# zhenyuw16/Uni3DETR

Measured on AMD Instinct MI355X. Metric: scenes/sec (fwd+bwd) SUN-RGB-D 20k pts, 300 queries, higher is better.
Workload: dtype bf16

## Files before the change

include/u3d_hip.h:

```cpp
#ifndef U3D_HIP_H_
#define U3D_HIP_H_

#include <stddef.h>
#include <stdint.h>

#ifdef __cplusplus
extern "C" {
#endif

typedef struct ihipStream_t* u3d_stream;

enum {
  U3D_OK = 0,
  U3D_ERR_ARG = -1,
  U3D_ERR_UNSUPPORTED = -2,
  U3D_ERR_LAUNCH = -3,
  U3D_ERR_WORKSPACE = -4
};

enum { U3D_F32 = 0, U3D_BF16 = 1 };

int32_t u3d_version(void);
const char* u3d_strerror(int32_t code);

int32_t u3d_event_create(void** event);
int32_t u3d_event_record(void* event, int32_t external, u3d_stream s);
int32_t u3d_event_elapsed_ms(void* start, void* stop, float* ms);
int32_t u3d_event_destroy(void* event);

typedef struct u3d_bitgrid {
  void* words;
  void* prefix;
  int32_t batch, dz, dy, dx;
  int32_t layout;
  int32_t row_capacity;
} u3d_bitgrid;

int64_t u3d_bitgrid_nwords(int32_t batch, int32_t dz, int32_t dy, int32_t dx);
int64_t u3d_bitgrid_nwords_layout(int32_t batch, int32_t dz, int32_t dy, int32_t dx, int32_t layout);

int32_t u3d_bitgrid_mark(const u3d_bitgrid* g, const int32_t* coors, int32_t n, u3d_stream s);

int32_t u3d_bitgrid_mark_strided(const u3d_bitgrid* g, const int32_t* in_coors, const int32_t* n_dev,
                                 int32_t n_cap, const int32_t ksize[3], const int32_t stride[3],
                                 const int32_t pad[3], u3d_stream s);

int64_t u3d_bitgrid_scan_scratch(int64_t nwords);
int32_t u3d_bitgrid_scan(const u3d_bitgrid* g, void* scratch, u3d_stream s);

int32_t u3d_bitgrid_rank(const u3d_bitgrid* g, const int32_t* coors, int32_t n, int32_t* rank, u3d_stream s);

int32_t u3d_bitgrid_coords(const u3d_bitgrid* g, int32_t* coors_out, int32_t cap, u3d_stream s);

int32_t u3d_nbr_table(const u3d_bitgrid* target, const int32_t* q_coors, const int32_t* n_dev, int32_t n_cap,
                      const int32_t ksize[3], const int32_t stride[3], const int32_t pad[3], int32_t mode,
                      int32_t* nbr, int32_t ld, u3d_stream s);

int32_t u3d_dense_nbr_table(int32_t batch, const int32_t q_dims[3], const int32_t t_dims[3], const int32_t ksize[3],
                            const int32_t stride[3], const int32_t pad[3], int32_t mode, int32_t* nbr, int32_t ld,
                            u3d_stream s);

int64_t u3d_voxelize_hard_workspace(int32_t n_total, int32_t batch, int32_t max_pts_per_scene);
int32_t u3d_voxelize_hard(const float* points, const int32_t* scene_off, int32_t batch, int32_t n_total,
                          int32_t max_pts_per_scene, int32_t nfeat, const float voxel_size[3],
                          const float pc_range[6], int32_t max_points, int32_t max_voxels,
                          float* voxels, int32_t* coors, int32_t* num_points, float* mean,
                          int32_t* voxel_off, void* workspace, int64_t workspace_bytes, u3d_stream s);

int32_t u3d_voxelize_dynamic(const float* points, const int32_t* scene_off, int32_t batch, int32_t n_total, int32_t nfeat,
                             const float voxel_size[3], const float pc_range[6], int32_t* coors, u3d_stream s);
int32_t u3d_scatter_mean(const float* points, const int32_t* rank, int32_t n_total, int32_t nfeat, float* sums,
                         int32_t* counts, int32_t n_voxels, u3d_stream s);

int32_t u3d_spconv_fwd(const void* in, const void* w, const int32_t* nbr, int32_t ld, void* out,
                       const int32_t* n_out_dev, int32_t n_out_cap, int32_t cin, int32_t cout, int32_t kvol,
                       int32_t transpose_w, int32_t dtype, u3d_stream s);

int32_t u3d_igemm_fwd_bf16(const void* in, const void* w, const int32_t* nbr, int32_t ld, void* out,
                           const int32_t* n_out_dev, int32_t n_out_cap, int32_t cin, int32_t cout, int32_t kvol,
                           int32_t transpose_w, u3d_stream s);
int32_t u3d_igemm_fwd_add_bf16(const void* in, const void* w, const int32_t* nbr, int32_t ld, const void* addend, void* out,
                               const int32_t* n_out_dev, int32_t n_out_cap, int32_t cin, int32_t cout, int32_t kvol,
                               int32_t transpose_w, u3d_stream s);
int32_t u3d_linear_bf16(const void* x, const void* w, const float* bias, int32_t relu, void* out, const int32_t* m_dev,
                        int32_t m_cap, int32_t k, int32_t n, u3d_stream s);
int64_t u3d_bn_fold_job_bytes(void);
int32_t u3d_bn_fold_job_blocks(int32_t kvol, int32_t cout, int32_t cin);
int32_t u3d_bn_fold_batched(const void* jobs, int32_t njobs, int32_t total_blocks, u3d_stream s);
int32_t u3d_igemm_fwd_affine_bf16(const void* in, const void* w_folded, const int32_t* nbr, int32_t ld, const float* shift, int32_t relu,
                                  void* out, const int32_t* n_out_dev, int32_t n_out_cap, int32_t cin, int32_t cout, int32_t kvol,
                                  u3d_stream s);
int32_t u3d_igemm_fwd_affine_plan(int32_t n_out_cap, int32_t cin, int32_t cout, int32_t kvol, int32_t has_nbr, int32_t* kernel,
                                  int32_t* rows, int32_t* cols);
int32_t u3d_igemm_fwd_split_bf16(const void* in, const void* w, const int32_t* nbr, int32_t ld, float* out, const int32_t* n_out_dev,
                                 int32_t n_out_cap, int32_t cin, int32_t cout, int32_t kvol3, double* stats, const float* addend, u3d_stream s);
int32_t u3d_igemm_direct_split_bf16(const void* in, const void* w3, const int32_t* nbr, int32_t ld, float* out, const int32_t* n_out_dev,
                                    int32_t n_out_cap, int32_t n_in_cap, int32_t cin, int32_t cout, u3d_stream s);
int32_t u3d_igemm_direct_affine_bf16(const void* in, const void* w_folded, const int32_t* nbr, int32_t ld, const float* shift,
                                     int32_t relu, const void* addend, void* out, const int32_t* n_out_dev, int32_t n_out_cap,
                                     int32_t cin, int32_t cout, u3d_stream s);
int32_t u3d_split3_weights(const float* src, int64_t sk, int64_t sa, int64_t sb, int32_t k, int32_t a, int32_t b, void* dst, u3d_stream s);
typedef struct U3dSplitRowsJobs {
  const float* src[32];
  void* dst[32];
  int32_t ld[32], rows[32], cols[32];
  int32_t first_block[33];
  int32_t njobs;
} U3dSplitRowsJobs;
int32_t u3d_split_rows_batch(const U3dSplitRowsJobs* jobs, u3d_stream s);
int32_t u3d_sum3_f32(const float* a, const float* b, const float* c, float* out, int64_t n, u3d_stream s);
int64_t u3d_split3_job_bytes(void);
int32_t u3d_split3_job_blocks(int32_t k, int32_t a, int32_t b);
int32_t u3d_split3_weights_batch(const void* jobs, int32_t njobs, int32_t total_blocks, u3d_stream s);
int32_t u3d_split_rows_f32(const float* x, const int32_t* n_dev, int32_t n_cap, int32_t c, void* dst, u3d_stream s);
int32_t u3d_igemm_fwd_stats_bf16(const void* in, const void* w, const int32_t* nbr, int32_t ld, void* out,
                                 const int32_t* n_out_dev, int32_t n_out_cap, int32_t cin, int32_t cout, int32_t kvol,
                                 double* stats, u3d_stream s);
int32_t u3d_igemm_fwd_stats_layout(int32_t n_out_cap, int32_t cin, int32_t cout, int32_t kvol, int32_t has_nbr, int32_t* partials,
                                   int32_t* rows_per_partial);
typedef struct {
  const void* x;
  const void* y;
  const float* mean;
  const float* invstd;
  const float* gamma;
  const float* beta;
  int32_t relu;
  int32_t reserved;
} u3d_bn_epi;
int32_t u3d_igemm_dgrad_bnstats_bf16(const void* in, const void* w, const int32_t* nbr, int32_t ld, const void* addend, void* out,
                                     const int32_t* n_out_dev, int32_t n_out_cap, int32_t cin, int32_t cout, int32_t kvol,
                                     const u3d_bn_epi* bn, double* stats, u3d_stream s);
int32_t u3d_bn_bwd_finalize_partials(const double* partial, int32_t nblocks, int32_t rows_per_block, const int32_t* n_dev,
                                     int32_t n_cap, int32_t c, double* sums, float* sums_f32, u3d_stream s);
int32_t u3d_subm_halo_sizes(int32_t n_cap, int64_t* tile_rows_elems, int64_t* loc_elems, int32_t* tiles);
int32_t u3d_subm_halo_build(const int32_t* nbr, int32_t ld, const int32_t* n_dev, int32_t n_cap, int32_t* tile_rows,
                            uint16_t* loc, int32_t* tile_cnt, int32_t kvol, u3d_stream s);
int32_t u3d_subm_halo_wpack(const void* w_nmajor, void* w_packed, u3d_stream s);
int32_t u3d_subm_halo_wpack_batched(const void* const* srcs_dev, void* const* dsts_dev, int32_t n, u3d_stream s);
int32_t u3d_subm_halo_conv64_bf16(const void* in, const void* w_packed, const int32_t* tile_rows, const uint16_t* loc,
                                  const int32_t* tile_cnt, const int32_t* n_dev, int32_t n_cap, int32_t krev,
                                  const void* addend, void* out, double* stats, const u3d_bn_epi* bn, int32_t max_slots,
                                  u3d_stream s);
int32_t u3d_subm_halo_wpack128(const void* w_nmajor, void* w_packed, int32_t kvol, u3d_stream s);
int32_t u3d_subm_halo_wpack128_batched(const void* const* srcs_dev, void* const* dsts_dev, int32_t n, int32_t kvol, u3d_stream s);
int32_t u3d_subm_halo_conv128_bf16(const void* in, const void* w_packed, const int32_t* tile_rows, const uint16_t* loc,
                                   const int32_t* tile_cnt, const int32_t* n_dev, int32_t n_cap, int32_t krev,
                                   const void* addend, void* out, double* stats, int32_t max_slots, int32_t kvol, u3d_stream s);
int32_t u3d_subm_halo_conv64_affine_bf16(const void* in, const void* w_packed, const int32_t* tile_rows, const uint16_t* loc,
                                         const int32_t* tile_cnt, const int32_t* n_dev, int32_t n_cap, const void* addend, void* out,
                                         const float* shift, int32_t relu, int32_t max_slots, u3d_stream s);
int32_t u3d_subm_halo_conv128_affine_bf16(const void* in, const void* w_packed, const int32_t* tile_rows, const uint16_t* loc,
                                          const int32_t* tile_cnt, const int32_t* n_dev, int32_t n_cap, const void* addend, void* out,
                                          const float* shift, int32_t relu, int32_t max_slots, int32_t kvol, u3d_stream s);
int64_t u3d_subm_halo_wgrad64_workspace(void);
int32_t u3d_subm_halo_wgrad64_bf16(const void* x, const void* dy, const int32_t* tile_rows, const uint16_t* loc,
                                   const int32_t* tile_cnt, const int32_t* n_dev, int32_t n_cap, float* dw, void* workspace,
                                   int64_t workspace_bytes, int32_t max_slots, u3d_stream s);
int64_t u3d_igemm_wgrad_bf16_workspace(int32_t n_out_cap, int32_t cin, int32_t cout, int32_t kvol);
int32_t u3d_igemm_wgrad_bf16(const void* in, const void* dout, const int32_t* nbr, int32_t ld, float* dw,
                             const int32_t* n_out_dev, int32_t n_out_cap, int32_t cin, int32_t cout, int32_t kvol,
                             int32_t out_layout, void* workspace, int64_t workspace_bytes, u3d_stream s);
int32_t u3d_igemm_wgrad_plan(int32_t n_out_cap, int32_t cin, int32_t cout, int32_t kvol, int32_t has_nbr, int32_t out_layout,
                             int32_t* kernel, int32_t* tile, int32_t* nsplit, int64_t* workspace);

int64_t u3d_spconv_wgrad_workspace(int32_t n_out_cap, int32_t cin, int32_t cout, int32_t kvol);
int32_t u3d_spconv_wgrad(const void* in, const void* dout, const int32_t* nbr, int32_t ld, float* dw,
                         const int32_t* n_out_dev, int32_t n_out_cap, int32_t cin, int32_t cout, int32_t kvol,
                         int32_t dtype, void* workspace, int64_t workspace_bytes, u3d_stream s);

int64_t u3d_colsum_workspace(int32_t n, int32_t c);
int32_t u3d_colsum(const void* x, int32_t n, int32_t c, int32_t dtype, float* out, void* workspace,
                   int64_t workspace_bytes, u3d_stream s);

int64_t u3d_wgrad_batched_workspace(int32_t count, int32_t n_rows, int32_t cin, int32_t cout);
int32_t u3d_wgrad_batched_bf16(const void* const* in, const void* const* dout, float* const* dw, int32_t count,
                               const int32_t* n_dev, int32_t n_rows, int32_t cin, int32_t cout, void* workspace,
                               int64_t workspace_bytes, u3d_stream s);
int64_t u3d_colsum_batched_workspace(int32_t count, int32_t n, int32_t c);
int32_t u3d_colsum_batched(const void* const* x, float* const* out, int32_t count, int32_t n, int32_t c, int32_t dtype,
                           void* workspace, int64_t workspace_bytes, u3d_stream s);

int32_t u3d_skinny_wgrad_chunks(int32_t m);
int32_t u3d_skinny_wgrad_bf16(const void* dy, const void* x, int32_t m, int32_t n, int32_t k, float* partial, u3d_stream s);
int32_t u3d_skinny_wgrad_batched(const void* const* dy, const void* const* x, float* const* partial, const int32_t* n, const int32_t* k,
                                 int32_t count, int32_t m, int32_t dy_skinny, u3d_stream s);

int64_t u3d_bn_stats_workspace(int32_t n_cap, int32_t c);
int32_t u3d_bn_stats(const void* x, const int32_t* n_dev, int32_t n_cap, int32_t c, int32_t dtype,
                     double* sums, void* workspace, int64_t workspace_bytes, u3d_stream s);
int32_t u3d_bn_finalize(const double* sums, const int32_t* n_dev, int32_t n_cap, int32_t c, float eps, float momentum,
                        float* running_mean, float* running_var, int64_t* num_batches, float* mean, float* invstd,
                        u3d_stream s);
int32_t u3d_bn_forward_stats(const void* x, const int32_t* n_dev, int32_t n_cap, int32_t c, int32_t dtype, float eps,
                             float momentum, float* running_mean, float* running_var, int64_t* num_batches, float* mean,
                             float* invstd, void* workspace, int64_t workspace_bytes, u3d_stream s);
int32_t u3d_bn_finalize_partials(const double* partial, int32_t nblocks, int32_t rows_per_block, const int32_t* n_dev,
                                 int32_t n_cap, int32_t c, float eps, float momentum, float* running_mean, float* running_var,
                                 int64_t* num_batches, float* mean, float* invstd, u3d_stream s);
int32_t u3d_bn_apply(const void* x, const float* mean, const float* invstd, const float* gamma,
                     const float* beta, const void* residual, int32_t relu, void* y,
                     const int32_t* n_dev, int32_t n_cap, int32_t c, int32_t dtype, const int32_t* row_map, const void* post_add,
                     u3d_stream s);
int32_t u3d_bn_bwd_stats(const void* dy, const void* y, const void* x, const float* mean, const float* invstd,
                         const float* gamma, const float* beta, int32_t relu, const int32_t* n_dev, int32_t n_cap,
                         int32_t c, int32_t dtype, double* sums, void* workspace, int64_t workspace_bytes,
                         const int32_t* row_map, float* sums_f32, u3d_stream s);
int32_t u3d_bn_bwd_apply(const void* dy, const void* y, const void* x, const float* mean, const float* invstd,
                         const float* gamma, const float* beta, const double* sums, int32_t relu, void* dx, void* dres,
                         const int32_t* n_dev, int32_t n_cap, int32_t c, int32_t dtype, const int32_t* row_map, u3d_stream s);
int32_t u3d_bn_apply_planes(const float* x, const float* mean, const float* invstd, const float* gamma, const float* beta,
                            const float* residual, int32_t relu, float* y, void* planes, const int32_t* n_dev, int32_t n_cap,
                            int32_t c, const int32_t* row_map, const float* post_add, u3d_stream s);
int32_t u3d_bn_bwd_apply_planes(const float* dy, const float* y, const float* x, const float* mean, const float* invstd,
                                const float* gamma, const float* beta, const double* sums, int32_t relu, float* dx, float* dres,
                                void* planes, const int32_t* n_dev, int32_t n_cap, int32_t c, const int32_t* row_map, u3d_stream s);

int32_t u3d_to_dense(const void* feat, const int32_t* coors, const int32_t* n_dev, int32_t n_cap, int32_t c,
                     void* dense, int32_t dz, int32_t dy, int32_t dx, int32_t dtype, u3d_stream s);
int32_t u3d_from_dense(const void* dense, const int32_t* coors, const int32_t* n_dev, int32_t n_cap, int32_t c,
                       void* feat, int32_t dz, int32_t dy, int32_t dx, int32_t dtype, u3d_stream s);

int32_t u3d_gather_rows(const void* in, const int32_t* idx, int32_t n, int32_t row_bytes, void* out, u3d_stream s);
int32_t u3d_scatter_rows(const void* in, const int32_t* idx, int32_t n, int32_t row_bytes, void* out, u3d_stream s);

int32_t u3d_fps(const float* base, const int64_t* set_off, const int32_t* set_n, int32_t nsets, int32_t max_n,
                int32_t m, int32_t* out_idx, float* temp, int64_t temp_stride, int32_t* err, int64_t poll_ticks, int32_t max_wg,
                u3d_stream s);
int32_t u3d_fps2(const float* base, const float* base2, int32_t split, const int64_t* set_off, const int32_t* set_n,
                 int32_t nsets, int32_t max_n, int32_t m, int32_t* out_idx, float* temp, int64_t temp_stride, int32_t* err,
                 int64_t poll_ticks, int32_t max_wg, u3d_stream s);
int32_t u3d_fps_prep(const int32_t* coors, int32_t v_rows, const int32_t* scene_off, const int32_t* voxel_off, int32_t batch,
                     int32_t nfeat, float* vox, int64_t* set_off, int32_t* set_n, u3d_stream s);
int32_t u3d_fps_points(const float* pts, int32_t nfeat, const float* vox, const int32_t* idx, const int32_t* scene_off,
                       const int32_t* voxel_off, int32_t batch, int32_t m, float* out, u3d_stream s);
int32_t u3d_query_embed_fwd(const float* tgt, const float* anchor, const float* fps, const float* rnd, int32_t batch, int32_t nq,
                            int32_t groups, int32_t c, float* query_embeds, float* query, float* ref, float* ref_sig, u3d_stream s);
int32_t u3d_query_embed_bwd(const float* d_query_embeds, const float* d_query, const float* d_ref, const float* d_ref_sig,
                            const float* anchor, int32_t batch, int32_t nq, int32_t groups, int32_t c, float* d_tgt, float* d_anchor,
                            u3d_stream s);

int32_t u3d_match_cost(const float* cls, const float* box, const float* gt, const int32_t* labels,
                       const int32_t* gt_off, int32_t nlayers, int32_t batch, int32_t nq_total, int32_t ncls,
                       int32_t code_size, int32_t gmax, float w_cls, float w_reg, float w_iou, float alpha,
                       float gamma, float* cost, u3d_stream s);
int32_t u3d_lsa(const float* cost, const int32_t* gt_off, int32_t nlayers, int32_t batch, int32_t nq_total,
                int32_t nq, int32_t gmax, int32_t* assigned, u3d_stream s);

int32_t u3d_trilinear_fwd(const void* value, const float* grid, int32_t batch, int32_t nq, int32_t dz, int32_t dy, int32_t dx,
                          int32_t c, void* out, int32_t dtype, u3d_stream s);
int32_t u3d_trilinear_bwd(const void* value, const float* grid, const void* dout, int32_t batch, int32_t nq, int32_t dz,
                          int32_t dy, int32_t dx, int32_t c, float* dvalue, float* dgrid, int32_t dtype, u3d_stream s);

int32_t u3d_iou3d_rotated_aligned(const float* a, const float* b, int32_t n, float* out, u3d_stream s);

int64_t u3d_nms3d_workspace(int32_t n);
int32_t u3d_nms3d(const float* boxes, const int32_t* labels, int32_t n, float thr, uint8_t* keep, void* workspace,
                  int64_t workspace_bytes, u3d_stream s);

#define U3D_DET_TAIL_NONE 0
#define U3D_DET_TAIL_NMS 1
#define U3D_DET_TAIL_DECODE 2
#define U3D_DET_TAIL_MAX_K 8192
#define U3D_DET_TAIL_LDS_CAP 2048
int64_t u3d_det_tail_workspace(int32_t batch, int32_t nq, int32_t num_classes, int32_t max_num, int32_t box_dim);
int32_t u3d_det_tail(const float* prob, const float* fused, const float* boxes, int32_t batch, int32_t nq, int32_t num_classes,
                     int32_t box_dim, int32_t max_num, const float* center_range, float score_threshold, int32_t mode, float nms_thr,
                     const float* score_thr, int32_t num_thr, float* out_boxes, float* out_scores, int32_t* out_labels,
                     int32_t* out_count, int32_t* out_off, void* workspace, int64_t workspace_bytes, u3d_stream s);

#define U3D_DET_TAIL_SOFT_NMS 3
#define U3D_DET_TAIL_MERGE 4
int64_t u3d_det_tail_pp_workspace(int32_t batch, int32_t nq, int32_t num_classes, int32_t max_num, int32_t box_dim, int32_t mode);
int32_t u3d_det_tail_pp(const float* prob, const float* fused, const float* boxes, int32_t batch, int32_t nq, int32_t num_classes,
                        int32_t box_dim, int32_t max_num, const float* center_range, float score_threshold, int32_t mode, float nms_thr,
                        const float* score_thr, int32_t num_thr, float soft_sigma, float soft_prune, float* out_boxes, float* out_scores,
                        int32_t* out_labels, int32_t* out_count, int32_t* out_off, void* workspace, int64_t workspace_bytes, u3d_stream s);

int32_t u3d_tap_gather_sum(const void* p, const int32_t* nbr, int32_t ld, const int32_t* n_dev, int32_t n_cap, int32_t c,
                           int32_t kvol, int32_t dtype, void* out, u3d_stream s);
int32_t u3d_tap_gather_sum_add(const void* p, const int32_t* nbr, int32_t ld, const int32_t* n_dev, int32_t n_cap, int32_t c,
                               int32_t kvol, int32_t dtype, const void* addend, void* out, u3d_stream s);

int32_t u3d_layernorm_blocks(int32_t n);
int32_t u3d_layernorm_fwd(const void* x, int32_t x_dtype, int32_t n, int32_t c, const float* gamma, const float* beta,
                          float eps, int32_t relu, void* y, int32_t y_dtype, float* mean, float* rstd, u3d_stream s);
int32_t u3d_layernorm_bwd(const void* dy, int32_t y_dtype, const void* x, int32_t x_dtype, int32_t n, int32_t c,
// ... 281 lines not shown
```

uni3detr_amd/csrc/geometry.hip:

```cpp
#include "common.h"

extern "C" int64_t u3d_bitgrid_nwords(int32_t batch, int32_t dz, int32_t dy, int32_t dx) {
  return (int64_t)batch * ((dz + 3) / 4) * ((dy + 3) / 4) * ((dx + 3) / 4);
}
extern "C" int64_t u3d_bitgrid_nwords_layout(int32_t batch, int32_t dz, int32_t dy, int32_t dx, int32_t layout) {
  if (layout == 1) return ((int64_t)batch * dz * dy * dx + 63) / 64;
  return u3d_bitgrid_nwords(batch, dz, dy, dx);
}
static inline long long grid_nwords(const u3d_bitgrid* g) { return u3d_bitgrid_nwords_layout(g->batch, g->dz, g->dy, g->dx, g->layout); }

__global__ void k_bitgrid_mark(BitGridDev g, unsigned long long* words, const int4* __restrict__ coors, int n) {
  int i = blockIdx.x * blockDim.x + threadIdx.x;
  if (i >= n) return;
  int4 c = coors[i];
  if (c.x < 0 || c.x >= g.B) return;
  if ((unsigned)c.y >= (unsigned)g.Dz || (unsigned)c.z >= (unsigned)g.Dy || (unsigned)c.w >= (unsigned)g.Dx) return;
  atomicOr(&words[u3d_word_index(g, c.x, c.y, c.z, c.w)], 1ull << u3d_bit_index(g, c.x, c.y, c.z, c.w));
}

extern "C" int32_t u3d_bitgrid_mark(const u3d_bitgrid* g, const int32_t* coors, int32_t n, u3d_stream s) {
  U3D_REQUIRE(g && g->words && coors, U3D_ERR_ARG);
  if (n <= 0) return U3D_OK;
  BitGridDev d = u3d_make_grid(g);
  hipLaunchKernelGGL(k_bitgrid_mark, dim3(u3d_cdiv(n, 256)), dim3(256), 0, s, d, (unsigned long long*)g->words,
// ... 188 lines not shown
  hipLaunchKernelGGL(k_scan_final, dim3(nchunks), dim3(SCAN_TPB), 0, s, (const unsigned long long*)g->words, nwords,
                     (const unsigned*)cs, (unsigned*)g->prefix, nchunks);
  U3D_CHECK_LAUNCH();
  return U3D_OK;
}

__global__ void k_bitgrid_rank(BitGridDev g, const int4* __restrict__ coors, int n, int* __restrict__ rank) {
  int i = blockIdx.x * blockDim.x + threadIdx.x;
  if (i >= n) return;
  int4 c = coors[i];
  rank[i] = (c.x < 0 || c.x >= g.B) ? -1 : u3d_grid_lookup(g, c.x, c.y, c.z, c.w);
}

extern "C" int32_t u3d_bitgrid_rank(const u3d_bitgrid* g, const int32_t* coors, int32_t n, int32_t* rank, u3d_stream s) {
  U3D_REQUIRE(g && g->words && g->prefix && coors && rank, U3D_ERR_ARG);
  if (n <= 0) return U3D_OK;
  hipLaunchKernelGGL(k_bitgrid_rank, dim3(u3d_cdiv(n, 256)), dim3(256), 0, s, u3d_make_grid(g), (const int4*)coors, n, rank);
  U3D_CHECK_LAUNCH();
  return U3D_OK;
}

__global__ void k_bitgrid_coords(BitGridDev g, long long nwords, int4* __restrict__ out, int cap) {
  long long w = (long long)blockIdx.x * blockDim.x + threadIdx.x;
  {
    const int count = g.prefix[nwords];
    for (long long i = w; i < cap; i += (long long)gridDim.x * blockDim.x)
      if (i >= count) out[i] = make_int4(-1, -1, -1, -1);
  }
  if (w >= nwords) return;
  unsigned long long bits = g.words[w];
  if (!bits) return;
  unsigned r = g.prefix[w];
  if (g.linear) {
    while (bits) {
      int bit = __ffsll((long long)bits) - 1;
      bits &= bits - 1;
      long long t = w * 64 + bit;
      int x = (int)(t % g.Dx); t /= g.Dx;
      int y = (int)(t % g.Dy); t /= g.Dy;
      int z = (int)(t % g.Dz); t /= g.Dz;
      if ((int)r < cap) out[r] = make_int4((int)t, z, y, x);
      ++r;
    }
    return;
  }
  long long t = w;
  int bx = (int)(t % g.bx); t /= g.bx;
  int by = (int)(t % g.by); t /= g.by;
  int bz = (int)(t % g.bz); t /= g.bz;
  int b = (int)t;
  while (bits) {
    int bit = __ffsll((long long)bits) - 1;
    bits &= bits - 1;
    if ((int)r < cap) out[r] = make_int4(b, bz * 4 + (bit >> 4), by * 4 + ((bit >> 2) & 3), bx * 4 + (bit & 3));
    ++r;
  }
}

extern "C" int32_t u3d_bitgrid_coords(const u3d_bitgrid* g, int32_t* coors_out, int32_t cap, u3d_stream s) {
  U3D_REQUIRE(g && g->words && g->prefix && coors_out, U3D_ERR_ARG);
  long long nwords = grid_nwords(g);
  hipLaunchKernelGGL(k_bitgrid_coords, dim3(u3d_cdiv(nwords, 256)), dim3(256), 0, s, u3d_make_grid(g), nwords,
                     (int4*)coors_out, cap);
  U3D_CHECK_LAUNCH();
  return U3D_OK;
}

__global__ void k_nbr_table(BitGridDev g, const int4* __restrict__ q, const int* __restrict__ n_dev, int n_cap,
                            Conv3 cv, int mode, int* __restrict__ nbr, int ld) {
  int i = blockIdx.x * blockDim.x + threadIdx.x;
  if (i >= ld) return;
  int n = min(*n_dev, n_cap);
  int kvol = cv.k[0] * cv.k[1] * cv.k[2];
  if (i >= n) {
    for (int k = 0; k < kvol; ++k) nbr[(long long)k * ld + i] = -1;
    return;
  }
  int4 c = q[i];
  int k = 0;
  for (int kz = 0; kz < cv.k[0]; ++kz)
    for (int ky = 0; ky < cv.k[1]; ++ky)
      for (int kx = 0; kx < cv.k[2]; ++kx, ++k) {
        int r = -1;
        if (mode == 0) {
          r = u3d_grid_lookup(g, c.x, c.y * cv.s[0] - cv.p[0] + kz, c.z * cv.s[1] - cv.p[1] + ky, c.w * cv.s[2] - cv.p[2] + kx);
        } else {
          int tz = c.y + cv.p[0] - kz, ty = c.z + cv.p[1] - ky, tx = c.w + cv.p[2] - kx;
          if (tz >= 0 && ty >= 0 && tx >= 0 && tz % cv.s[0] == 0 && ty % cv.s[1] == 0 && tx % cv.s[2] == 0)
            r = u3d_grid_lookup(g, c.x, tz / cv.s[0], ty / cv.s[1], tx / cv.s[2]);
        }
        nbr[(long long)k * ld + i] = r;
      }
}

extern "C" int32_t u3d_nbr_table(const u3d_bitgrid* target, const int32_t* q_coors, const int32_t* n_dev, int32_t n_cap,
                                 const int32_t ksize[3], const int32_t stride[3], const int32_t pad[3], int32_t mode,
                                 int32_t* nbr, int32_t ld, u3d_stream s) {
  U3D_REQUIRE(target && target->words && target->prefix && q_coors && n_dev && nbr, U3D_ERR_ARG);
  U3D_REQUIRE(ld >= n_cap && (mode == 0 || mode == 1), U3D_ERR_ARG);
  if (ld <= 0) return U3D_OK;
  Conv3 cv;
  for (int i = 0; i < 3; ++i) { cv.k[i] = ksize[i]; cv.s[i] = stride[i]; cv.p[i] = pad[i]; U3D_REQUIRE(stride[i] > 0 && ksize[i] > 0, U3D_ERR_ARG); }
  hipLaunchKernelGGL(k_nbr_table, dim3(u3d_cdiv(ld, 256)), dim3(256), 0, s, u3d_make_grid(target), (const int4*)q_coors,
                     n_dev, n_cap, cv, mode, nbr, ld);
  U3D_CHECK_LAUNCH();
  return U3D_OK;
}

__global__ void k_dense_nbr_table(int B, int qz, int qy, int qx, int tz, int ty, int tx, Conv3 cv, int mode,
                                  int* __restrict__ nbr, int ld) {
  int i = blockIdx.x * blockDim.x + threadIdx.x;
  if (i >= ld) return;
  int kvol = cv.k[0] * cv.k[1] * cv.k[2];
  long long nq = (long long)B * qz * qy * qx;
  if (i >= nq) {
    for (int k = 0; k < kvol; ++k) nbr[(long long)k * ld + i] = -1;
    return;
  }
  int x = i % qx; int t = i / qx;
  int y = t % qy; t /= qy;
  int z = t % qz; int b = t / qz;
  int k = 0;
  for (int kz = 0; kz < cv.k[0]; ++kz)
    for (int ky = 0; ky < cv.k[1]; ++ky)
      for (int kx = 0; kx < cv.k[2]; ++kx, ++k) {
        int pz, py, px;
        bool ok = true;
        if (mode == 0) {
          pz = z * cv.s[0] - cv.p[0] + kz; py = y * cv.s[1] - cv.p[1] + ky; px = x * cv.s[2] - cv.p[2] + kx;
        } else {
          int uz = z + cv.p[0] - kz, uy = y + cv.p[1] - ky, ux = x + cv.p[2] - kx;
          ok = uz >= 0 && uy >= 0 && ux >= 0 && uz % cv.s[0] == 0 && uy % cv.s[1] == 0 && ux % cv.s[2] == 0;
          pz = uz / cv.s[0]; py = uy / cv.s[1]; px = ux / cv.s[2];
        }
        ok = ok && (unsigned)pz < (unsigned)tz && (unsigned)py < (unsigned)ty && (unsigned)px < (unsigned)tx;
        nbr[(long long)k * ld + i] = ok ? (int)((((long long)b * tz + pz) * ty + py) * tx + px) : -1;
      }
}

extern "C" int32_t u3d_dense_nbr_table(int32_t batch, const int32_t q_dims[3], const int32_t t_dims[3], const int32_t ksize[3],
                                       const int32_t stride[3], const int32_t pad[3], int32_t mode, int32_t* nbr, int32_t ld,
                                       u3d_stream s) {
  U3D_REQUIRE(nbr && batch > 0 && (mode == 0 || mode == 1), U3D_ERR_ARG);
  long long nq = (long long)batch * q_dims[0] * q_dims[1] * q_dims[2];
  U3D_REQUIRE(ld >= nq && nq < 0x7fffffffll, U3D_ERR_ARG);
  Conv3 cv;
  for (int i = 0; i < 3; ++i) { cv.k[i] = ksize[i]; cv.s[i] = stride[i]; cv.p[i] = pad[i]; U3D_REQUIRE(stride[i] > 0 && ksize[i] > 0, U3D_ERR_ARG); }
  hipLaunchKernelGGL(k_dense_nbr_table, dim3(u3d_cdiv(ld, 256)), dim3(256), 0, s, batch, q_dims[0], q_dims[1], q_dims[2],
                     t_dims[0], t_dims[1], t_dims[2], cv, mode, nbr, ld);
  U3D_CHECK_LAUNCH();
  return U3D_OK;
}

__global__ void k_gather_rows(const uint32_t* __restrict__ in, const int* __restrict__ idx, int n, int row_words,
                              uint32_t* __restrict__ out) {
  long long t = (long long)blockIdx.x * blockDim.x + threadIdx.x;
  long long total = (long long)n * row_words;
  if (t >= total) return;
  int r = (int)(t / row_words), w = (int)(t % row_words);
  int src = idx[r];
  out[t] = src >= 0 ? in[(long long)src * row_words + w] : 0u;
}
__global__ void k_scatter_rows(const uint32_t* __restrict__ in, const int* __restrict__ idx, int n, int row_words,
                               uint32_t* __restrict__ out) {
  long long t = (long long)blockIdx.x * blockDim.x + threadIdx.x;
  long long total = (long long)n * row_words;
  if (t >= total) return;
  int r = (int)(t / row_words), w = (int)(t % row_words);
  int dst = idx[r];
  if (dst >= 0) out[(long long)dst * row_words + w] = in[t];
}

extern "C" int32_t u3d_gather_rows(const void* in, const int32_t* idx, int32_t n, int32_t row_bytes, void* out, u3d_stream s) {
  U3D_REQUIRE(in && idx && out && row_bytes > 0 && (row_bytes & 3) == 0, U3D_ERR_ARG);
  if (n <= 0) return U3D_OK;
  int rw = row_bytes / 4;
  hipLaunchKernelGGL(k_gather_rows, dim3(u3d_cdiv((long long)n * rw, 256)), dim3(256), 0, s, (const uint32_t*)in, idx, n, rw, (uint32_t*)out);
  U3D_CHECK_LAUNCH();
  return U3D_OK;
}
extern "C" int32_t u3d_scatter_rows(const void* in, const int32_t* idx, int32_t n, int32_t row_bytes, void* out, u3d_stream s) {
  U3D_REQUIRE(in && idx && out && row_bytes > 0 && (row_bytes & 3) == 0, U3D_ERR_ARG);
  if (n <= 0) return U3D_OK;
  int rw = row_bytes / 4;
  hipLaunchKernelGGL(k_scatter_rows, dim3(u3d_cdiv((long long)n * rw, 256)), dim3(256), 0, s, (const uint32_t*)in, idx, n, rw, (uint32_t*)out);
  U3D_CHECK_LAUNCH();
  return U3D_OK;
}

struct VoxCfg {
  float vs[3], lo[3];
  int grid[3];
  int nfeat, max_points, max_voxels, hsize;
};

__device__ __forceinline__ unsigned hash_u32(unsigned k) {
  k ^= k >> 16; k *= 0x7feb352dU; k ^= k >> 15; k *= 0x846ca68bU; k ^= k >> 16;
  return k;
}

__global__ void k_vox_insert(const float* __restrict__ pts, const int* __restrict__ scene_off, int B, int n_total, VoxCfg cfg,
                             unsigned* __restrict__ keys, unsigned* __restrict__ first, int* __restrict__ head,
                             int* __restrict__ next, int* __restrict__ slot_of) {
  int i = blockIdx.x * blockDim.x + threadIdx.x;
  if (i >= n_total) return;
  if (i >= scene_off[B]) { slot_of[i] = -1; next[i] = -1; return; }
  int b = 0;
  while (b + 1 < B && i >= scene_off[b + 1]) ++b;
  int il = i - scene_off[b];
  const float* p = pts + (long long)i * cfg.nfeat;
  int c[3];
  bool ok = true;
#pragma unroll
  for (int j = 0; j < 3; ++j) {
    float q = __fdiv_rn(__fsub_rn(p[j], cfg.lo[j]), cfg.vs[j]);
    bool in = (q >= 0.f) && (q < (float)cfg.grid[j]);
    c[j] = in ? (int)floorf(q) : 0;
    ok = ok && in;
  }
  if (!ok) { slot_of[i] = -1; next[i] = -1; return; }
  unsigned key = ((unsigned)c[2] * (unsigned)cfg.grid[1] + (unsigned)c[1]) * (unsigned)cfg.grid[0] + (unsigned)c[0];
  unsigned mask = (unsigned)cfg.hsize - 1u;
  unsigned h = hash_u32(key) & mask;
  long long tb = (long long)b * cfg.hsize;
  while (true) {
    unsigned prev = atomicCAS(&keys[tb + h], 0xFFFFFFFFu, key);
    if (prev == 0xFFFFFFFFu || prev == key) break;
    h = (h + 1) & mask;
  }
  atomicMin(&first[tb + h], (unsigned)il);
  next[i] = atomicExch(&head[tb + h], il);
  slot_of[i] = (int)h;
}

__global__ void k_vox_rank(const int* __restrict__ scene_off, VoxCfg cfg, const unsigned* __restrict__ first,
                           const int* __restrict__ slot_of, int* __restrict__ vid, int* __restrict__ scene_cnt) {
  __shared__ unsigned wsum[16];
  __shared__ unsigned carry_s;
  int b = blockIdx.x;
  int p0 = scene_off[b], n = scene_off[b + 1] - p0;
  long long tb = (long long)b * cfg.hsize;
  if (threadIdx.x == 0) carry_s = 0;
  __syncthreads();
  int lane = threadIdx.x & 63, wid = threadIdx.x >> 6;
  for (int base = 0; base < n; base += 1024) {
    int il = base + threadIdx.x;
    int sl = -1;
    unsigned flag = 0;
    if (il < n) {
      sl = slot_of[p0 + il];
      if (sl >= 0 && first[tb + sl] == (unsigned)il) flag = 1;
    }
    unsigned long long bal = __ballot(flag);
    unsigned in_wave = __popcll(bal & ((1ull << lane) - 1ull));
    if (lane == 0) wsum[wid] = __popcll(bal);
    __syncthreads();
    unsigned woff = 0, tot = 0;
    for (int w = 0; w < 16; ++w) { unsigned v = wsum[w]; if (w < wid) woff += v; tot += v; }
    unsigned carry = carry_s;
    if (flag) {
      unsigned r = carry + woff + in_wave;
      vid[tb + sl] = (r < (unsigned)cfg.max_voxels) ? (int)r : -1;
    }
    __syncthreads();
    if (threadIdx.x == 0) carry_s = carry + tot;
    __syncthreads();
  }
  if (threadIdx.x == 0) scene_cnt[b] = (int)min(carry_s, (unsigned)cfg.max_voxels);
}

__global__ void k_vox_offsets(const int* __restrict__ scene_cnt, int B, int* __restrict__ voxel_off) {
  if (threadIdx.x == 0 && blockIdx.x == 0) {
    int acc = 0;
    for (int b = 0; b < B; ++b) { voxel_off[b] = acc; acc += scene_cnt[b]; }
    voxel_off[B] = acc;
  }
}

__global__ void k_vox_write(const float* __restrict__ pts, const int* __restrict__ scene_off, int B, int n_total, VoxCfg cfg,
                            const unsigned* __restrict__ keys, const unsigned* __restrict__ first, const int* __restrict__ head,
                            const int* __restrict__ next, const int* __restrict__ slot_of, const int* __restrict__ vid,
                            const int* __restrict__ voxel_off, float* __restrict__ voxels, int4* __restrict__ coors,
                            int* __restrict__ num_points, float* __restrict__ mean) {
  int i = blockIdx.x * blockDim.x + threadIdx.x;
  if (i >= n_total || i >= scene_off[B]) return;
  int sl = slot_of[i];
  if (sl < 0) return;
  int b = 0;
  while (b + 1 < B && i >= scene_off[b + 1]) ++b;
  int p0 = scene_off[b];
  int il = i - p0;
  long long tb = (long long)b * cfg.hsize;
  if (first[tb + sl] != (unsigned)il) return;
  int v = vid[tb + sl];
  if (v < 0) return;
  long long row = (long long)voxel_off[b] + v;
  unsigned key = keys[tb + sl];
  int cx = (int)(key % (unsigned)cfg.grid[0]);
  unsigned t = key / (unsigned)cfg.grid[0];
  int cy = (int)(t % (unsigned)cfg.grid[1]);
  int cz = (int)(t / (unsigned)cfg.grid[1]);
  coors[row] = make_int4(b, cz, cy, cx);
  int last = -1, cnt = 0;
  float acc[8];
  const int nf = cfg.nfeat;
  for (int f = 0; f < 8; ++f) acc[f] = 0.f;
// ... 151 lines not shown
```

uni3detr_amd/csrc/igemm_bf16.hip:

```cpp
#include "igemm_common.h"
#include "conv_in.h"
#include "igemm_direct.h"

struct BnEpi {
  const u16* x = nullptr;
  const u16* y = nullptr;
  const float *mean = nullptr, *invstd = nullptr, *gamma = nullptr, *beta = nullptr;
  int relu = 0, pad = 0;
};
template <int BM, int BN, int NT>
__device__ __forceinline__ void bn_bwd_tile_sums(const BnEpi bn, u16* smem, int m0, int col0, int n_out, int cout, int tile,
                                              double* __restrict__ stats, int tid) {
  constexpr int CPR = BN / 8, SWZ = (CPR - 1) & 15, R = NT / CPR, ROWS = BM / R, BATCH = ROWS < 8 ? ROWS : (ROWS % 8 == 0 ? 8 : (ROWS % 6 == 0 ? 6 : 4));
  static_assert(NT % CPR == 0 && BM % R == 0 && ROWS % BATCH == 0, "tile / thread mismatch");
  const int cc = tid % CPR, r0 = tid / CPR;
  const int col = col0 + cc * 8;
  const bool from_y = bn.relu && bn.y, remask = bn.relu && !bn.y;
  float s0[8], s1[8], mu[8], is[8], ga[8], be[8];
#pragma unroll
  for (int e = 0; e < 8; ++e) { s0[e] = 0.f; s1[e] = 0.f; mu[e] = 0.f; is[e] = 0.f; ga[e] = 0.f; be[e] = 0.f; }
  __syncthreads();
  if (col < cout) {
#pragma unroll
    for (int e = 0; e < 8; ++e) { mu[e] = bn.mean[col + e]; is[e] = bn.invstd[col + e]; }
// ... 276 lines not shown
  const int nstage = kvol * kchunks;

  f32x4 acc[WM][WN];
#pragma unroll
  for (int a = 0; a < WM; ++a)
#pragma unroll
    for (int b = 0; b < WN; ++b) acc[a][b] = (f32x4){0.f, 0.f, 0.f, 0.f};

  const __amdgpu_buffer_rsrc_t in_rs = __builtin_amdgcn_make_buffer_rsrc((void*)in, 0, -1, 0x00020000);
  const __amdgpu_buffer_rsrc_t w_rs = __builtin_amdgcn_make_buffer_rsrc((void*)w, 0, -1, 0x00020000);
  const unsigned row_bytes = (unsigned)cin * 2u;
  const int lrow = lane >> 3, lslot = lane & 7;
  unsigned a_part16[SEGS_A], w_voff[SEGS_W];
  int arow[SEGS_A];
#pragma unroll
  for (int u = 0; u < SEGS_A; ++u) {
    const int r = (wv * SEGS_A + u) * 8 + lrow;
    arow[u] = r;
    a_part16[u] = (unsigned)(lslot ^ ((r >> 1) & 7)) * 16u;
  }
#pragma unroll
  for (int u = 0; u < SEGS_W; ++u) {
    const int r = (wv * SEGS_W + u) * 8 + lrow;
    const int part = lslot ^ ((r >> 1) & 7);
    w_voff[u] = (col0 + r < cout) ? (unsigned)((col0 + r) * cin + part * 8) * 2u : 0xFFFFFFFFu;
  }
  int idx_cur[SEGS_A], idx_nxt[SEGS_A];
  auto load_idx_next = [&](int stage) {
    const int kap = stage % kvol;
#pragma unroll
    for (int u = 0; u < SEGS_A; ++u) {
      int m = m0 + arow[u];
      int mc = m < n_out ? m : n_out - 1;
      idx_nxt[u] = nbr ? nbr[(long long)kap * ld + mc] : mc;
    }
  };
  auto advance_idx = [&]() {
#pragma unroll
    for (int u = 0; u < SEGS_A; ++u) idx_cur[u] = (m0 + arow[u] < n_out) ? idx_nxt[u] : -1;
  };
  auto issue = [&](int st, int buf) {
    const int kap = st % kvol, c0 = (st / kvol) * BK;
    u16* Ab = smem + buf * STAGE_ELEMS + wv * (SEGS_A * 512);
    u16* Wb = smem + buf * STAGE_ELEMS + A_ELEMS + wv * (SEGS_W * 512);
    const unsigned a_soff = (unsigned)c0 * 2u;
    const unsigned w_soff = (unsigned)(kap * cin * cout + c0) * 2u;
#pragma unroll
    for (int u = 0; u < SEGS_A; ++u) {
      unsigned voff = idx_cur[u] >= 0 ? (unsigned)idx_cur[u] * row_bytes + a_part16[u] : 0xFFFFFFFFu;
      __builtin_amdgcn_raw_ptr_buffer_load_lds(in_rs, (lds_void_ptr)(Ab + u * 512), 16, voff, a_soff, 0, 0);
    }
#pragma unroll
    for (int u = 0; u < SEGS_W; ++u)
      __builtin_amdgcn_raw_ptr_buffer_load_lds(w_rs, (lds_void_ptr)(Wb + u * 512), 16, w_voff[u], w_soff, 0, 0);
  };
#if GLDS_FRAG_B128
  auto issue_one = [&](int st, int buf, int q) {
    const int kap = st % kvol, c0 = (st / kvol) * BK;
    if (q < SEGS_A) {
      u16* Ab = smem + buf * STAGE_ELEMS + wv * (SEGS_A * 512);
      unsigned voff = idx_cur[q] >= 0 ? (unsigned)idx_cur[q] * row_bytes + a_part16[q] : 0xFFFFFFFFu;
      __builtin_amdgcn_raw_ptr_buffer_load_lds(in_rs, (lds_void_ptr)(Ab + q * 512), 16, voff, (unsigned)c0 * 2u, 0, 0);
    } else {
      const int u = q - SEGS_A;
      u16* Wb = smem + buf * STAGE_ELEMS + A_ELEMS + wv * (SEGS_W * 512);
      __builtin_amdgcn_raw_ptr_buffer_load_lds(w_rs, (lds_void_ptr)(Wb + u * 512), 16, w_voff[u], (unsigned)(kap * cin * cout + c0) * 2u, 0, 0);
    }
  };
  const int g = lane >> 4, li = lane & 15, fsw = (lane >> 1) & 7;
  int foff[2];
#pragma unroll
  for (int ks = 0; ks < 2; ++ks) foff[ks] = ((ks * 4 + g) ^ fsw) << 3;
  typedef const volatile s16x8 __attribute__((address_space(3))) * lds_vptr;
  auto frag = [&](const u16* rowp, int ks) {
    s16x8 v = *(lds_vptr)(rowp + foff[ks]);
    return __builtin_bit_cast(bf16x8, v);
  };
#else
  const int g = lane >> 4, li = lane & 15, fsw = (lane >> 1) & 7;
  int foff[2][2];
#pragma unroll
  for (int ks = 0; ks < 2; ++ks)
#pragma unroll
    for (int j = 0; j < 2; ++j) foff[ks][j] = (((ks * 4 + (g >> 1) + 2 * j) ^ fsw) << 3) + (g & 1) * 4;
  typedef const volatile s16x4 __attribute__((address_space(3))) * lds_vptr;
  auto frag = [&](const u16* rowp, int ks) {
    s16x4 x = *(lds_vptr)(rowp + foff[ks][0]);
    s16x4 y = *(lds_vptr)(rowp + foff[ks][1]);
    s16x8 v = {x[0], x[1], x[2], x[3], y[0], y[1], y[2], y[3]};
    return __builtin_bit_cast(bf16x8, v);
  };

#endif
  load_idx_next(0);
  advance_idx();
  load_idx_next(1 < nstage ? 1 : 0);
  issue(0, 0);
  __syncthreads();
  for (int st = 0; st < nstage; ++st) {
    const int buf = st & 1;
    const int nx = st + 1 < nstage ? st + 1 : st;
    advance_idx();
    load_idx_next(st + 2 < nstage ? st + 2 : nstage - 1);
#if !GLDS_DMA_SPREAD
    issue(nx, buf ^ 1);
#endif
    const u16* A = smem + buf * STAGE_ELEMS + (wm * WM * 16 + li) * BK;
    const u16* W = smem + buf * STAGE_ELEMS + A_ELEMS + (wn * WN * 16 + li) * BK;
#pragma unroll
    for (int ks = 0; ks < 2; ++ks) {
      bf16x8 af[WM];
#pragma unroll
      for (int a = 0; a < WM; ++a) af[a] = frag(A + a * 16 * BK, ks);
#pragma unroll
      for (int b = 0; b < WN; ++b) {
        bf16x8 bfr = frag(W + b * 16 * BK, ks);
#pragma unroll
        for (int a = 0; a < WM; ++a) acc[a][b] = __builtin_amdgcn_mfma_f32_16x16x32_bf16(bfr, af[a], acc[a][b], 0, 0, 0);
#if GLDS_DMA_SPREAD
        {
          constexpr int NQ = SEGS_A + SEGS_W, NG = (GLDS_DMA_SPREAD == 1) ? 2 * WN : (GLDS_DMA_SPREAD == 3 ? (WN > 1 ? WN / 2 : 1) : (GLDS_DMA_SPREAD == 4 ? WN + WN / 2 : WN));
          constexpr int PER = (NQ + NG - 1) / NG;
          const int grp = ks * WN + b;
          if (grp < NG) {
#pragma unroll
            for (int j = 0; j < PER; ++j)
              if (grp * PER + j < NQ) issue_one(nx, buf ^ 1, grp * PER + j);
          }
          __builtin_amdgcn_sched_barrier(0);
        }
#endif
      }
    }
    __syncthreads();
  }
#define GLDS_EPI_ADDEND (BM != 256 || BN != 256)
#include "glds_epilogue.inc"
#undef GLDS_EPI_ADDEND
}

#ifndef GLDS8_PRIO
#define GLDS8_PRIO 1
#endif
#ifndef GLDS8_BALANCE
#define GLDS8_BALANCE 1
#endif
#ifndef GLDS8_STAGGER
#define GLDS8_STAGGER 1
#endif
template <bool F32OUT = false, int RB = 4>
__device__ __forceinline__ void igemm_glds8_body(const u16* __restrict__ in, const u16* __restrict__ w, const int* __restrict__ nbr,
                                                 int ld, u16* __restrict__ out, const int* __restrict__ n_out_dev, int n_out_cap,
                                                 int cin, int cout, int kvol, const float* __restrict__ bias, int relu,
                                                 double* __restrict__ stats, const BnEpi bn) {
  constexpr int WAVES_M = 2, WAVES_N = 4, WM = 2 * RB, WN = 4, NW = 8;
  constexpr int BM = 64 * RB, BN = 256, BK = 64;
  constexpr int PIECE = 128 * BK;
  constexpr int STAGE_ELEMS = 4 * PIECE;
  extern __shared__ __attribute__((aligned(16))) u16 smem[];

  const int n_out = min(*n_out_dev, n_out_cap);
  const int tile = u3d_xcd_tile(blockIdx.x, (n_out + BM - 1) / BM);
  if (tile < 0) return;
  const int m0 = tile * BM;
  const int col0 = blockIdx.y * BN;
  const int tid = threadIdx.x, lane = tid & 63;
  const int wv = __builtin_amdgcn_readfirstlane(tid >> 6);
  const int wm = wv / WAVES_N, wn = wv % WAVES_N;
  const int nstage = kvol * (cin / BK);

  f32x4 acc[WM][WN];
#pragma unroll
  for (int a = 0; a < WM; ++a)
#pragma unroll
    for (int b = 0; b < WN; ++b) acc[a][b] = (f32x4){0.f, 0.f, 0.f, 0.f};

  const __amdgpu_buffer_rsrc_t in_rs = __builtin_amdgcn_make_buffer_rsrc((void*)in, 0, -1, 0x00020000);
  const __amdgpu_buffer_rsrc_t w_rs = __builtin_amdgcn_make_buffer_rsrc((void*)w, 0, -1, 0x00020000);
  const unsigned row_bytes = (unsigned)cin * 2u;
  const int lrow = lane >> 3, lslot = lane & 7;
  unsigned a_part16[2], w_voff[2][2];
  int arow[2][2];
#pragma unroll
  for (int u = 0; u < 2; ++u) {
    const int r = (wv * 2 + u) * 8 + lrow;
    a_part16[u] = (unsigned)(lslot ^ ((r >> 1) & 7)) * 16u;
#pragma unroll
    for (int sp = 0; sp < 2; ++sp) {
      arow[sp][u] = ((r & 63) < 16 * RB) ? (r >> 6) * (32 * RB) + sp * (16 * RB) + (r & 63) : -1;
      const int tc = (r >> 5) * 64 + sp * 32 + (r & 31);
      w_voff[sp][u] = (col0 + tc < cout) ? (unsigned)((col0 + tc) * cin + (lslot ^ ((r >> 1) & 7)) * 8) * 2u : 0xFFFFFFFFu;
    }
  }
  int idx_cur[2][2], idx_nxt[2][2];
  int mcl[2][2];
#pragma unroll
  for (int sp = 0; sp < 2; ++sp)
#pragma unroll
    for (int u = 0; u < 2; ++u) {
      const int m = m0 + (arow[sp][u] < 0 ? 0 : arow[sp][u]);
      mcl[sp][u] = m < n_out ? m : n_out - 1;
      idx_nxt[sp][u] = mcl[sp][u];
    }
  auto load_idx_next = [&](int stage) {
    const int* row = nbr + (long long)(stage % kvol) * ld;
#pragma unroll
    for (int sp = 0; sp < 2; ++sp)
#pragma unroll
      for (int u = 0; u < 2; ++u) idx_nxt[sp][u] = row[mcl[sp][u]];
  };
  auto advance_idx = [&]() {
#pragma unroll
    for (int sp = 0; sp < 2; ++sp)
#pragma unroll
      for (int u = 0; u < 2; ++u) idx_cur[sp][u] = (arow[sp][u] >= 0 && m0 + arow[sp][u] < n_out) ? idx_nxt[sp][u] : -1;
  };
  auto issue_a = [&](int st, int buf, int sp) {
    const unsigned soff = (unsigned)((st / kvol) * BK) * 2u;
    u16* dst = smem + buf * STAGE_ELEMS + sp * PIECE + wv * 1024;
#pragma unroll
    for (int u = 0; u < 2; ++u) {
      const unsigned voff = idx_cur[sp][u] >= 0 ? (unsigned)idx_cur[sp][u] * row_bytes + a_part16[u] : 0xFFFFFFFFu;
      __builtin_amdgcn_raw_ptr_buffer_load_lds(in_rs, (lds_void_ptr)(dst + u * 512), 16, voff, soff, 0, 0);
    }
  };
  auto issue_b = [&](int st, int buf, int sp) {
    const unsigned soff = (unsigned)((st % kvol) * cin * cout + (st / kvol) * BK) * 2u;
    u16* dst = smem + buf * STAGE_ELEMS + (2 + sp) * PIECE + wv * 1024;
#pragma unroll
    for (int u = 0; u < 2; ++u)
      __builtin_amdgcn_raw_ptr_buffer_load_lds(w_rs, (lds_void_ptr)(dst + u * 512), 16, w_voff[sp][u], soff, 0, 0);
  };
  const int g = lane >> 4, li = lane & 15, fsw = (lane >> 1) & 7;
  int foff[2];
#pragma unroll
  for (int ks = 0; ks < 2; ++ks) foff[ks] = ((ks * 4 + g) ^ fsw) << 3;
  typedef const volatile s16x8 __attribute__((address_space(3))) * lds_vptr;
  auto frag = [&](const u16* rowp, int ks) {
    s16x8 v = *(lds_vptr)(rowp + foff[ks]);
    return __builtin_bit_cast(bf16x8, v);
  };
#if GLDS8_BALANCE
  bf16x8 af2[2][RB][2], bf[2][2][2];
#define G8_AF(SP) af2[SP]
#else
  bf16x8 af1[RB][2], bf[2][2][2];
#define G8_AF(SP) af1
#endif
#define G8_READ_A(BUF, SP)                                                                                   \
  {                                                                                                          \
    const u16* A_ = smem + (BUF) * STAGE_ELEMS + (SP) * PIECE + (wm * 64 + li) * BK;                         \
    _Pragma("unroll") for (int a = 0; a < RB; ++a) {                                                         \
      G8_AF(SP)[a][0] = frag(A_ + a * 16 * BK, 0);                                                           \
      G8_AF(SP)[a][1] = frag(A_ + a * 16 * BK, 1);                                                           \
    }                                                                                                        \
  }
#define G8_READ_B(BUF, SP)                                                                                   \
  {                                                                                                          \
    const u16* B_ = smem + (BUF) * STAGE_ELEMS + (2 + (SP)) * PIECE + (wn * 32 + li) * BK;                   \
    _Pragma("unroll") for (int b = 0; b < 2; ++b) {                                                          \
      bf[SP][b][0] = frag(B_ + b * 16 * BK, 0);                                                              \
      bf[SP][b][1] = frag(B_ + b * 16 * BK, 1);                                                              \
    }                                                                                                        \
  }
#define G8_MMA(SA, SB)                                                                                       \
  {                                                                                                          \
    __builtin_amdgcn_s_setprio(GLDS8_PRIO);                                                                  \
    _Pragma("unroll") for (int ks = 0; ks < 2; ++ks)                                                         \
      _Pragma("unroll") for (int b = 0; b < 2; ++b)                                                          \
        _Pragma("unroll") for (int a = 0; a < RB; ++a)                                                       \
          acc[(SA) * RB + a][(SB) * 2 + b] =                                                                 \
              __builtin_amdgcn_mfma_f32_16x16x32_bf16(bf[SB][b][ks], G8_AF(SA)[a][ks], acc[(SA) * RB + a][(SB) * 2 + b], 0, 0, 0); \
    __builtin_amdgcn_s_setprio(0);                                                                           \
  }
#define G8_BAR()                                  \
  {                                               \
    __builtin_amdgcn_sched_barrier(0);            \
    __builtin_amdgcn_s_barrier();                 \
    __builtin_amdgcn_sched_barrier(0);            \
  }
#define G8_VMCNT8() __builtin_amdgcn_s_waitcnt(0x0F78)

  load_idx_next(0);
  advance_idx();
  issue_a(0, 0, 0); issue_b(0, 0, 0); issue_b(0, 0, 1); issue_a(0, 0, 1);
  load_idx_next(1 < nstage ? 1 : 0);
  advance_idx();
  __builtin_amdgcn_s_waitcnt(0x0F70);
  G8_BAR();
#if GLDS8_BALANCE
  G8_READ_A(0, 0)
#endif
  if (GLDS8_STAGGER && wm == 1) G8_BAR();
  for (int st = 0; st < nstage; ++st) {
    const int buf = st & 1;
    const int nx = st + 1 < nstage ? st + 1 : st;
    load_idx_next(st + 2 < nstage ? st + 2 : nstage - 1);
    __builtin_amdgcn_sched_barrier(0);
    G8_READ_B(buf, 0)
#if !GLDS8_BALANCE
    __builtin_amdgcn_sched_barrier(0);
    G8_READ_A(buf, 0)
#endif
    issue_a(nx, buf ^ 1, 0);
    G8_VMCNT8();
    G8_BAR();
    G8_MMA(0, 0)
    G8_BAR();
    G8_READ_B(buf, 1)
    issue_b(nx, buf ^ 1, 0);
    G8_VMCNT8();
    G8_BAR();
    G8_MMA(0, 1)
    G8_BAR();
    G8_READ_A(buf, 1)
    issue_b(nx, buf ^ 1, 1);
#if GLDS8_BALANCE
    __builtin_amdgcn_s_waitcnt(0x0F74);
#endif
    G8_BAR();
    G8_MMA(1, 1)
    G8_BAR();
#if GLDS8_BALANCE
    G8_READ_A(buf ^ 1, 0)
#endif
    issue_a(nx, buf ^ 1, 1);
    __builtin_amdgcn_sched_barrier(0);
    advance_idx();
    __builtin_amdgcn_s_waitcnt(0x0F74);
    G8_BAR();
    G8_MMA(1, 0)
    G8_BAR();
  }
  if (GLDS8_STAGGER && wm == 0) G8_BAR();
  __builtin_amdgcn_s_waitcnt(0x0F70);
  __syncthreads();
#undef G8_AF
#undef G8_READ_A
#undef G8_READ_B
#undef G8_MMA
#undef G8_BAR
#undef G8_VMCNT8
#define GLDS_EPI_ADDEND 1
#include "glds_epilogue.inc"
#undef GLDS_EPI_ADDEND
}
__global__ __launch_bounds__(512) void k_igemm_glds8_256x256(const u16* in, const u16* w, const int* nbr, int ld, u16* out,
                                                             const int* n_out_dev, int n_out_cap, int cin, int cout, int kvol,
                                                             const float* bias, int relu, double* stats, BnEpi bn) {
  igemm_glds8_body(in, w, nbr, ld, out, n_out_dev, n_out_cap, cin, cout, kvol, bias, relu, stats, bn);
}
__global__ __launch_bounds__(512) void k_igemm_glds8_256x256_f32o(const u16* in, const u16* w, const int* nbr, int ld, u16* out,
                                                                  const int* n_out_dev, int n_out_cap, int cin, int cout, int kvol,
                                                                  const float* bias, int relu, double* stats, BnEpi bn) {
  igemm_glds8_body<true>(in, w, nbr, ld, out, n_out_dev, n_out_cap, cin, cout, kvol, bias, relu, stats, bn);
}
__global__ __launch_bounds__(512) void k_igemm_glds8_192x256(const u16* in, const u16* w, const int* nbr, int ld, u16* out,
                                                             const int* n_out_dev, int n_out_cap, int cin, int cout, int kvol,
                                                             const float* bias, int relu, double* stats, BnEpi bn) {
  igemm_glds8_body<false, 3>(in, w, nbr, ld, out, n_out_dev, n_out_cap, cin, cout, kvol, bias, relu, stats, bn);
}
__global__ __launch_bounds__(512) void k_igemm_glds8_192x256_f32o(const u16* in, const u16* w, const int* nbr, int ld, u16* out,
                                                                  const int* n_out_dev, int n_out_cap, int cin, int cout, int kvol,
                                                                  const float* bias, int relu, double* stats, BnEpi bn) {
  igemm_glds8_body<true, 3>(in, w, nbr, ld, out, n_out_dev, n_out_cap, cin, cout, kvol, bias, relu, stats, bn);
}
static inline bool igemm_rows192(int n_out_cap, int col_blocks) {
  const long long w256 = (long long)u3d_cdiv(n_out_cap, 256) * col_blocks, w192 = (long long)u3d_cdiv(n_out_cap, 192) * col_blocks;
  return (double)u3d_cdiv(w192, 256) * 192.0 * 1.05 < (double)u3d_cdiv(w256, 256) * 256.0;
}

template <bool F32OUT = false, int RB = 4>
__device__ __forceinline__ void igemm_glds8n_body(const u16* __restrict__ in, const u16* __restrict__ w, const int* __restrict__ nbr,
                                                  int ld, u16* __restrict__ out, const int* __restrict__ n_out_dev, int n_out_cap,
                                                  int cin, int cout, int kvol, const float* __restrict__ bias, int relu,
                                                  double* __restrict__ stats, const BnEpi bn) {
  constexpr int WAVES_M = 4, WAVES_N = 2, WM = RB, WN = 4, NW = 8;
  constexpr int BM = 64 * RB, BN = 128, BK = 64;
  constexpr int APIECE = 128 * BK, BPIECE = 64 * BK;
  constexpr int STAGE_ELEMS = 2 * APIECE + 2 * BPIECE;
  extern __shared__ __attribute__((aligned(16))) u16 smem[];

  const int n_out = min(*n_out_dev, n_out_cap);
  const int tile = u3d_xcd_tile(blockIdx.x, (n_out + BM - 1) / BM);
  if (tile < 0) return;
  const int m0 = tile * BM;
  const int col0 = blockIdx.y * BN;
  const int tid = threadIdx.x, lane = tid & 63;
  const int wv = __builtin_amdgcn_readfirstlane(tid >> 6);
  const int grp = wv >> 2, wm = wv >> 1, wn = wv & 1;
  const int nstage = kvol * (cin / BK);

  f32x4 acc[WM][WN];
#pragma unroll
  for (int a = 0; a < WM; ++a)
#pragma unroll
    for (int b = 0; b < WN; ++b) acc[a][b] = (f32x4){0.f, 0.f, 0.f, 0.f};

  const __amdgpu_buffer_rsrc_t in_rs = __builtin_amdgcn_make_buffer_rsrc((void*)in, 0, -1, 0x00020000);
  const __amdgpu_buffer_rsrc_t w_rs = __builtin_amdgcn_make_buffer_rsrc((void*)w, 0, -1, 0x00020000);
  const unsigned row_bytes = (unsigned)cin * 2u;
  const int lrow = lane >> 3, lslot = lane & 7;
  unsigned a_part16[2], w_voff[2];
  int arow[2][2];
#pragma unroll
  for (int u = 0; u < 2; ++u) {
    const int r = (wv * 2 + u) * 8 + lrow;
    a_part16[u] = (unsigned)(lslot ^ ((r >> 1) & 7)) * 16u;
#pragma unroll
    for (int gp = 0; gp < 2; ++gp) arow[gp][u] = ((r & 63) < 16 * RB) ? gp * (32 * RB) + (r >> 6) * (16 * RB) + (r & 63) : -1;
  }
  {
    const int r = wv * 8 + lrow;
#pragma unroll
    for (int t = 0; t < 2; ++t) {
      const int tc = (r >> 5) * 64 + t * 32 + (r & 31);
      w_voff[t] = (col0 + tc < cout) ? (unsigned)((col0 + tc) * cin + (lslot ^ ((r >> 1) & 7)) * 8) * 2u : 0xFFFFFFFFu;
    }
  }
  int idx_cur[2][2], idx_nxt[2][2], mcl[2][2];
#pragma unroll
  for (int gp = 0; gp < 2; ++gp)
#pragma unroll
    for (int u = 0; u < 2; ++u) {
      const int m = m0 + (arow[gp][u] < 0 ? 0 : arow[gp][u]);
      mcl[gp][u] = m < n_out ? m : n_out - 1;
      idx_nxt[gp][u] = mcl[gp][u];
    }
  auto load_idx_next = [&](int stage) {
    const int* row = nbr + (long long)(stage % kvol) * ld;
#pragma unroll
    for (int gp = 0; gp < 2; ++gp)
#pragma unroll
      for (int u = 0; u < 2; ++u) idx_nxt[gp][u] = row[mcl[gp][u]];
  };
  auto advance_idx = [&]() {
#pragma unroll
    for (int gp = 0; gp < 2; ++gp)
#pragma unroll
      for (int u = 0; u < 2; ++u) idx_cur[gp][u] = (arow[gp][u] >= 0 && m0 + arow[gp][u] < n_out) ? idx_nxt[gp][u] : -1;
  };
  auto issue_a = [&](int st, int sl) {
    const unsigned soff = (unsigned)((st / kvol) * BK) * 2u;
#pragma unroll
    for (int gp = 0; gp < 2; ++gp) {
      u16* dst = smem + sl * STAGE_ELEMS + gp * APIECE + wv * 1024;
#pragma unroll
      for (int u = 0; u < 2; ++u) {
        const unsigned voff = idx_cur[gp][u] >= 0 ? (unsigned)idx_cur[gp][u] * row_bytes + a_part16[u] : 0xFFFFFFFFu;
        __builtin_amdgcn_raw_ptr_buffer_load_lds(in_rs, (lds_void_ptr)(dst + u * 512), 16, voff, soff, 0, 0);
      }
    }
  };
  auto issue_b = [&](int st, int sl) {
    const unsigned soff = (unsigned)((st % kvol) * cin * cout + (st / kvol) * BK) * 2u;
#pragma unroll
    for (int t = 0; t < 2; ++t) {
      u16* dst = smem + sl * STAGE_ELEMS + 2 * APIECE + t * BPIECE + wv * 512;
      __builtin_amdgcn_raw_ptr_buffer_load_lds(w_rs, (lds_void_ptr)dst, 16, w_voff[t], soff, 0, 0);
    }
  };
  const int g = lane >> 4, li = lane & 15, fsw = (lane >> 1) & 7;
  int foff[2];
#pragma unroll
  for (int ks = 0; ks < 2; ++ks) foff[ks] = ((ks * 4 + g) ^ fsw) << 3;
  typedef const volatile s16x8 __attribute__((address_space(3))) * lds_vptr;
  auto frag = [&](const u16* rowp, int ks) {
    s16x8 v = *(lds_vptr)(rowp + foff[ks]);
    return __builtin_bit_cast(bf16x8, v);
  };
  bf16x8 af[2][RB][2], bf[2][2][2];
#define N8_READ_A(SL, SET)                                                                                   \
  {                                                                                                          \
    const u16* A_ = smem + (SL) * STAGE_ELEMS + grp * APIECE + (((wv >> 1) & 1) * 64 + li) * BK;             \
    _Pragma("unroll") for (int a = 0; a < RB; ++a) {                                                         \
      af[SET][a][0] = frag(A_ + a * 16 * BK, 0);                                                             \
      af[SET][a][1] = frag(A_ + a * 16 * BK, 1);                                                             \
    }                                                                                                        \
  }
#define N8_READ_B(SL)                                                                                        \
  {                                                                                                          \
    _Pragma("unroll") for (int t = 0; t < 2; ++t) {                                                          \
      const u16* B_ = smem + (SL) * STAGE_ELEMS + 2 * APIECE + t * BPIECE + (wn * 32 + li) * BK;             \
      _Pragma("unroll") for (int b = 0; b < 2; ++b) {                                                        \
        bf[t][b][0] = frag(B_ + b * 16 * BK, 0);                                                             \
        bf[t][b][1] = frag(B_ + b * 16 * BK, 1);                                                             \
      }                                                                                                      \
    }                                                                                                        \
  }
#define N8_MMA(SET, T)                                                                                       \
  {                                                                                                          \
    __builtin_amdgcn_s_setprio(1);                                                                           \
    _Pragma("unroll") for (int ks = 0; ks < 2; ++ks)                                                         \
      _Pragma("unroll") for (int b = 0; b < 2; ++b)                                                          \
        _Pragma("unroll") for (int a = 0; a < RB; ++a)                                                       \
          acc[a][(T) * 2 + b] =                                                                              \
              __builtin_amdgcn_mfma_f32_16x16x32_bf16(bf[T][b][ks], af[SET][a][ks], acc[a][(T) * 2 + b], 0, 0, 0); \
    __builtin_amdgcn_s_setprio(0);                                                                           \
  }
#define N8_BAR()                                  \
  {                                               \
    __builtin_amdgcn_sched_barrier(0);            \
    __builtin_amdgcn_s_barrier();                 \
    __builtin_amdgcn_sched_barrier(0);            \
  }
#define N8_TRIP(SET)                                                                                         \
  {                                                                                                          \
    const int s2 = st + 2 < nstage ? st + 2 : nstage - 1;                                                    \
    load_idx_next(st + 3 < nstage ? st + 3 : nstage - 1);                                                    \
    __builtin_amdgcn_sched_barrier(0);                                                                       \
    N8_READ_B(sl0)                                                                                           \
    issue_a(s2, sl2);                                                                                        \
    __builtin_amdgcn_s_waitcnt(0x0F7A);                                   \
    N8_BAR();                                                                                                \
    N8_MMA(SET, 0)                                                                                           \
    N8_BAR();                                                                                                \
    N8_READ_A(sl1, (SET) ^ 1)                                                                                \
    issue_b(s2, sl2);                                                                                        \
    __builtin_amdgcn_sched_barrier(0);                                                                       \
    advance_idx();                                                                                           \
    __builtin_amdgcn_s_waitcnt(0x0F7A);                                   \
    N8_BAR();                                                                                                \
    N8_MMA(SET, 1)                                                                                           \
    N8_BAR();                                                                                                \
    { const int t_ = sl0; sl0 = sl1; sl1 = sl2; sl2 = t_; }                                                  \
    ++st;                                                                                                    \
  }
  load_idx_next(0);
  advance_idx();
  issue_a(0, 0); issue_b(0, 0);
  load_idx_next(1 < nstage ? 1 : 0);
  advance_idx();
  issue_a(1 < nstage ? 1 : 0, 1); issue_b(1 < nstage ? 1 : 0, 1);
  load_idx_next(2 < nstage ? 2 : nstage - 1);
  advance_idx();
  __builtin_amdgcn_s_waitcnt(0x0F70);
  N8_BAR();
  N8_READ_A(0, 0)
  if (grp == 1) N8_BAR();
  int st = 0, sl0 = 0, sl1 = 1, sl2 = 2;
  while (st + 1 < nstage) {
    N8_TRIP(0)
    N8_TRIP(1)
  }
  if (st < nstage) N8_TRIP(0)
  if (grp == 0) N8_BAR();
  __builtin_amdgcn_s_waitcnt(0x0F70);
  __syncthreads();
#undef N8_READ_A
#undef N8_READ_B
#undef N8_MMA
#undef N8_BAR
#undef N8_TRIP
#define GLDS_EPI_ADDEND 1
#include "glds_epilogue.inc"
#undef GLDS_EPI_ADDEND
}
__global__ __launch_bounds__(512) void k_igemm_glds8_256x128(const u16* in, const u16* w, const int* nbr, int ld, u16* out,
                                                             const int* n_out_dev, int n_out_cap, int cin, int cout, int kvol,
                                                             const float* bias, int relu, double* stats, BnEpi bn) {
  igemm_glds8n_body(in, w, nbr, ld, out, n_out_dev, n_out_cap, cin, cout, kvol, bias, relu, stats, bn);
}
__global__ __launch_bounds__(512) void k_igemm_glds8_256x128_f32o(const u16* in, const u16* w, const int* nbr, int ld, u16* out,
                                                                  const int* n_out_dev, int n_out_cap, int cin, int cout, int kvol,
                                                                  const float* bias, int relu, double* stats, BnEpi bn) {
  igemm_glds8n_body<true>(in, w, nbr, ld, out, n_out_dev, n_out_cap, cin, cout, kvol, bias, relu, stats, bn);
}
__global__ __launch_bounds__(512) void k_igemm_glds8_192x128(const u16* in, const u16* w, const int* nbr, int ld, u16* out,
                                                             const int* n_out_dev, int n_out_cap, int cin, int cout, int kvol,
                                                             const float* bias, int relu, double* stats, BnEpi bn) {
  igemm_glds8n_body<false, 3>(in, w, nbr, ld, out, n_out_dev, n_out_cap, cin, cout, kvol, bias, relu, stats, bn);
}
__global__ __launch_bounds__(512) void k_igemm_glds8_192x128_f32o(const u16* in, const u16* w, const int* nbr, int ld, u16* out,
                                                                  const int* n_out_dev, int n_out_cap, int cin, int cout, int kvol,
                                                                  const float* bias, int relu, double* stats, BnEpi bn) {
  igemm_glds8n_body<true, 3>(in, w, nbr, ld, out, n_out_dev, n_out_cap, cin, cout, kvol, bias, relu, stats, bn);
}
#define U3D_GLDS_KERNEL(NAME, A, B, C, D)                                                                                        \
  __global__ __launch_bounds__(A* B * 64) void NAME(const u16* in, const u16* w, const int* nbr, int ld, u16* out,               \
                                                    const int* n_out_dev, int n_out_cap, int cin, int cout, int kvol,            \
                                                    const float* bias, int relu, double* stats, BnEpi bn) {                      \
    igemm_glds_body<A, B, C, D>(in, w, nbr, ld, out, n_out_dev, n_out_cap, cin, cout, kvol, bias, relu, stats, bn);               \
  }
#define U3D_GLDS_KERNEL_X(NAME, ...) U3D_GLDS_KERNEL(NAME, __VA_ARGS__)
U3D_GLDS_KERNEL_X(k_igemm_glds_256x256, GLDS256_CFG)
U3D_GLDS_KERNEL(k_igemm_glds_256x128, 4, 2, 4, 4)
U3D_GLDS_KERNEL(k_igemm_glds_128x64, 4, 1, 2, 4)
U3D_GLDS_KERNEL(k_igemm_glds_128x128, 2, 2, 4, 4)
#undef U3D_GLDS_KERNEL
#define U3D_GLDS_KERNEL_F32O(NAME, A, B, C, D)                                                                                   \
  __global__ __launch_bounds__(A* B * 64) void NAME(const u16* in, const u16* w, const int* nbr, int ld, u16* out,               \
                                                    const int* n_out_dev, int n_out_cap, int cin, int cout, int kvol,            \
                                                    const float* bias, int relu, double* stats, BnEpi bn) {                      \
    igemm_glds_body<A, B, C, D, true>(in, w, nbr, ld, out, n_out_dev, n_out_cap, cin, cout, kvol, bias, relu, stats, bn);         \
  }
U3D_GLDS_KERNEL_F32O(k_igemm_glds_128x64_f32o, 4, 1, 2, 4)
U3D_GLDS_KERNEL_F32O(k_igemm_glds_128x128_f32o, 2, 2, 4, 4)
#undef U3D_GLDS_KERNEL_F32O
typedef void (*glds_kernel_t)(const u16*, const u16*, const int*, int, u16*, const int*, int, int, int, int, const float*, int, double*, BnEpi);


struct GldsKernel {
  glds_kernel_t bf16, f32;
  int rows, cols, threads;
  size_t lds;
  bool addend;
};
#define GLDS_GEOM(A, B, C, D) A * C * 16, B * D * 16, A * B * 64, (size_t)2 * (A * C * 16 + B * D * 16) * 64 * 2
#define GLDS_GEOM_X(...) GLDS_GEOM(__VA_ARGS__)
enum { G_256x256, G8_256x256, G8_192x256, G8_256x128, G8_192x128, G_256x128, G_128x128, G_128x64, G_COUNT };
static const GldsKernel GLDS_KERNELS[G_COUNT] = {
    {k_igemm_glds_256x256, nullptr, GLDS_GEOM_X(GLDS256_CFG), false},
    {k_igemm_glds8_256x256, k_igemm_glds8_256x256_f32o, 256, 256, 512, 2 * (256 + 256) * 64 * 2, true},
    {k_igemm_glds8_192x256, k_igemm_glds8_192x256_f32o, 192, 256, 512, 2 * (256 + 256) * 64 * 2, true},
    {k_igemm_glds8_256x128, k_igemm_glds8_256x128_f32o, 256, 128, 512, 3 * (256 + 128) * 64 * 2, true},
    {k_igemm_glds8_192x128, k_igemm_glds8_192x128_f32o, 192, 128, 512, 3 * (256 + 128) * 64 * 2, true},
    {k_igemm_glds_256x128, nullptr, GLDS_GEOM(4, 2, 4, 4), true},
    {k_igemm_glds_128x128, k_igemm_glds_128x128_f32o, GLDS_GEOM(2, 2, 4, 4), true},
    {k_igemm_glds_128x64, k_igemm_glds_128x64_f32o, GLDS_GEOM(4, 1, 2, 4), true},
};
#undef GLDS_GEOM_X
#undef GLDS_GEOM

enum FwdEpi { EPI_PLAIN, EPI_BIAS_RELU, EPI_ADD, EPI_F32, EPI_F32_ADD, EPI_STATS, EPI_BN_BWD, EPI_AFFINE };

struct FwdPlan {
  DirectPlan direct;
  glds_kernel_t fn = nullptr;
  int glds = -1, rows = 0;
  dim3 grid;
  int threads = 0;
  size_t lds = 0;
  int partials = 0;
  bool served() const { return fn || direct.slot >= 0; }
};

constexpr int GLDS8N_MIN_KTILES = 48;
constexpr int GLDS8N_MIN_WGS = 160;

static FwdPlan fwd_plan(int n_out_cap, int cin, int cout, int kvol, bool has_nbr, bool nmajor, FwdEpi epi) {
  FwdPlan p;
  if (epi == EPI_PLAIN || epi == EPI_ADD || epi == EPI_STATS) {
    p.direct = u3d_plan_igemm_direct(n_out_cap, cin, cout, kvol, has_nbr, nmajor, epi == EPI_STATS ? DIR_STATS : DIR_BF16);
    if (p.direct.slot >= 0) {
      p.partials = p.direct.partials;
      return p;
    }
  }
  if (!nmajor || cin <= 0 || cout <= 0 || cin % 64 != 0 || cout % 64 != 0 || n_out_cap <= 0) return p;
  const long long tiles256 = u3d_cdiv(n_out_cap, 256);
  const bool r192 = has_nbr && kvol > 1;
  int g;
  if (epi == EPI_BIAS_RELU)
    g = (cout % 256 == 0 && tiles256 * (cout / 256) >= 128) ? G_256x256
        : (cout % 128 == 0 && tiles256 * (cout / 128) >= 128) ? G_256x128 : G_128x64;
  else if (cout % 256 == 0 && tiles256 * (cout / 256) >= 128)
    g = !has_nbr ? G_256x256 : (r192 && igemm_rows192(n_out_cap, cout / 256)) ? G8_192x256 : G8_256x256;
  else if (has_nbr && cout % 128 == 0 && kvol * (cin / 64) >= GLDS8N_MIN_KTILES && tiles256 * (cout / 128) >= GLDS8N_MIN_WGS)
    g = (r192 && igemm_rows192(n_out_cap, cout / 128)) ? G8_192x128 : G8_256x128;
  else
    g = cout % 128 == 0 ? G_128x128 : G_128x64;
  const GldsKernel& k = GLDS_KERNELS[g];
  const bool f32 = epi == EPI_F32 || epi == EPI_F32_ADD;
  if (!k.addend && (epi == EPI_ADD || epi == EPI_F32_ADD || epi == EPI_BN_BWD)) return p;
  p.fn = f32 ? k.f32 : k.bf16;
  if (!p.fn) return p;
  p.glds = g;
  p.rows = k.rows;
  p.grid = dim3(u3d_cdiv(n_out_cap, k.rows), u3d_cdiv(cout, k.cols));
  p.threads = k.threads;
  p.lds = k.lds;
  p.partials = (int)p.grid.x;
  return p;
}

static int fwd_launch(const FwdPlan& p, const void* in, const void* w, const int32_t* nbr, int ld, void* out, const int32_t* n_out_dev,
                      int n_out_cap, int cin, int cout, int kvol, hipStream_t s, const void* bias = nullptr, int relu = 0,
                      double* stats = nullptr, const BnEpi bn = BnEpi{}) {
  if (p.direct.slot >= 0) return u3d_launch_igemm_direct(p.direct, in, w, nbr, ld, out, n_out_dev, n_out_cap, cin, cout, s, bias, stats);
  static unsigned long long lds_mask[G_COUNT][2] = {};
  if (p.lds > 64 * 1024) u3d_allow_lds_impl((const void*)p.fn, (int)p.lds, &lds_mask[p.glds][p.fn == GLDS_KERNELS[p.glds].f32]);
  hipLaunchKernelGGL(p.fn, p.grid, dim3(p.threads), p.lds, s, (const u16*)in, (const u16*)w, nbr, ld, (u16*)out, n_out_dev, n_out_cap, cin,
                     cout, kvol, (const float*)bias, relu, stats, bn);
  return hipGetLastError() == hipSuccess ? U3D_OK : U3D_ERR_LAUNCH;
}

extern "C" int32_t u3d_linear_bf16(const void* x, const void* w, const float* bias, int32_t relu, void* out,
                                   const int32_t* m_dev, int32_t m_cap, int32_t k, int32_t n, u3d_stream s) {
  U3D_REQUIRE(x && w && out && m_dev, U3D_ERR_ARG);
  if (k % 64 != 0 || n % 64 != 0) return U3D_ERR_UNSUPPORTED;
  if (m_cap <= 0) return U3D_OK;
  const FwdPlan p = fwd_plan(m_cap, k, n, 1, false, true, EPI_BIAS_RELU);
  if (!p.served()) return U3D_ERR_UNSUPPORTED;
  return fwd_launch(p, x, w, nullptr, 0, out, m_dev, m_cap, k, n, 1, s, bias, relu ? 1 : 0);
}

extern "C" int32_t u3d_igemm_fwd_affine_bf16(const void* in, const void* w_folded, const int32_t* nbr, int32_t ld, const float* shift,
                                             int32_t relu, void* out, const int32_t* n_out_dev, int32_t n_out_cap, int32_t cin,
                                             int32_t cout, int32_t kvol, u3d_stream s) {
  U3D_REQUIRE(in && w_folded && out && n_out_dev && shift && kvol > 0 && (nbr || kvol == 1), U3D_ERR_ARG);
  if (cin <= 0 || cout <= 0 || cin % 64 != 0 || cout % 64 != 0) return U3D_ERR_UNSUPPORTED;
  if (n_out_cap <= 0) return U3D_OK;
  const FwdPlan p = fwd_plan(n_out_cap, cin, cout, kvol, nbr != nullptr, true, EPI_AFFINE);
  if (!p.served()) return U3D_ERR_UNSUPPORTED;
  return fwd_launch(p, in, w_folded, nbr, ld, out, n_out_dev, n_out_cap, cin, cout, kvol, s, shift, relu ? 1 : 0);
}
extern "C" int32_t u3d_igemm_fwd_affine_plan(int32_t n_out_cap, int32_t cin, int32_t cout, int32_t kvol, int32_t has_nbr, int32_t* kernel,
                                             int32_t* rows, int32_t* cols) {
  U3D_REQUIRE(kernel && rows && cols, U3D_ERR_ARG);
  const FwdPlan p = fwd_plan(n_out_cap, cin, cout, kvol, has_nbr != 0, true, EPI_AFFINE);
  if (!p.served()) return U3D_ERR_UNSUPPORTED;
  *kernel = p.glds;
  *rows = p.rows;
  *cols = GLDS_KERNELS[p.glds].cols;
  return U3D_OK;
}

extern "C" int32_t u3d_igemm_fwd_stats_layout(int32_t n_out_cap, int32_t cin, int32_t cout, int32_t kvol, int32_t has_nbr, int32_t* partials,
                                              int32_t* rows_per_partial) {
  U3D_REQUIRE(partials && rows_per_partial, U3D_ERR_ARG);
  const FwdPlan p = fwd_plan(n_out_cap, cin, cout, kvol, has_nbr != 0, true, EPI_STATS);
  if (!p.served()) return U3D_ERR_UNSUPPORTED;
  *partials = p.partials;
  *rows_per_partial = p.rows;
  return U3D_OK;
}
extern "C" int32_t u3d_igemm_fwd_stats_bf16(const void* in, const void* w, const int32_t* nbr, int32_t ld, void* out,
                                            const int32_t* n_out_dev, int32_t n_out_cap, int32_t cin, int32_t cout, int32_t kvol,
                                            double* stats, u3d_stream s) {
  U3D_REQUIRE(in && w && out && n_out_dev && stats && (nbr || kvol == 1), U3D_ERR_ARG);
  const FwdPlan p = fwd_plan(n_out_cap, cin, cout, kvol, nbr != nullptr, true, EPI_STATS);
  if (!p.served()) return U3D_ERR_UNSUPPORTED;
  return fwd_launch(p, in, w, nbr, ld, out, n_out_dev, n_out_cap, cin, cout, kvol, s, nullptr, 0, stats);
}

extern "C" int32_t u3d_igemm_fwd_split_bf16(const void* in, const void* w, const int32_t* nbr, int32_t ld, float* out,
                                            const int32_t* n_out_dev, int32_t n_out_cap, int32_t cin, int32_t cout, int32_t kvol3,
                                            double* stats, const float* addend, u3d_stream s) {
  U3D_REQUIRE(in && w && out && n_out_dev && nbr && kvol3 > 0, U3D_ERR_ARG);
  if (cin % 64 != 0 || cout % 64 != 0) return U3D_ERR_UNSUPPORTED;
  if (n_out_cap <= 0) return U3D_OK;
  const FwdPlan p = fwd_plan(n_out_cap, cin, cout, kvol3, true, true, addend ? EPI_F32_ADD : EPI_F32);
  if (!p.served()) return U3D_ERR_UNSUPPORTED;
  return fwd_launch(p, in, w, nbr, ld, out, n_out_dev, n_out_cap, cin, cout, kvol3, s, addend, addend ? 2 : 0, stats);
}


extern "C" int32_t u3d_igemm_fwd_add_bf16(const void* in, const void* w, const int32_t* nbr, int32_t ld, const void* addend, void* out,
                                          const int32_t* n_out_dev, int32_t n_out_cap, int32_t cin, int32_t cout, int32_t kvol,
                                          int32_t transpose_w, u3d_stream s) {
  U3D_REQUIRE(in && w && out && addend && n_out_dev && nbr, U3D_ERR_ARG);
  if (n_out_cap <= 0) return U3D_OK;
  const FwdPlan p = fwd_plan(n_out_cap, cin, cout, kvol, true, transpose_w != 0, EPI_ADD);
  if (!p.served()) return U3D_ERR_UNSUPPORTED;
  return fwd_launch(p, in, w, nbr, ld, out, n_out_dev, n_out_cap, cin, cout, kvol, s, addend, 2);
}

extern "C" int32_t u3d_igemm_dgrad_bnstats_bf16(const void* in, const void* w, const int32_t* nbr, int32_t ld, const void* addend, void* out,
                                                const int32_t* n_out_dev, int32_t n_out_cap, int32_t cin, int32_t cout, int32_t kvol,
                                                const u3d_bn_epi* bn, double* stats, u3d_stream s) {
  U3D_REQUIRE(in && w && out && n_out_dev && nbr && bn && bn->x && bn->mean && bn->invstd && stats, U3D_ERR_ARG);
  U3D_REQUIRE(!bn->relu || bn->y || (bn->gamma && bn->beta), U3D_ERR_ARG);
  const FwdPlan p = fwd_plan(n_out_cap, cin, cout, kvol, true, true, EPI_BN_BWD);
  if (!p.served()) return U3D_ERR_UNSUPPORTED;
  BnEpi e;
  e.x = (const u16*)bn->x; e.y = (const u16*)bn->y; e.mean = bn->mean; e.invstd = bn->invstd; e.gamma = bn->gamma; e.beta = bn->beta;
  e.relu = bn->relu;
  return fwd_launch(p, in, w, nbr, ld, out, n_out_dev, n_out_cap, cin, cout, kvol, s, addend, addend ? 2 : 0, stats, e);
}

extern "C" int32_t u3d_igemm_fwd_bf16(const void* in, const void* w, const int32_t* nbr, int32_t ld, void* out,
                                      const int32_t* n_out_dev, int32_t n_out_cap, int32_t cin, int32_t cout, int32_t kvol,
                                      int32_t transpose_w, u3d_stream s) {
  U3D_REQUIRE(in && w && out && n_out_dev && (nbr || kvol == 1), U3D_ERR_ARG);
  if (!transpose_w && convin_shape(cin, cout, kvol))
    return u3d_launch_conv_in_fwd(in, w, nbr, ld, out, n_out_dev, n_out_cap, kvol, s);
  const FwdPlan p = fwd_plan(n_out_cap, cin, cout, kvol, nbr != nullptr, transpose_w != 0, EPI_PLAIN);
  if (p.served()) return fwd_launch(p, in, w, nbr, ld, out, n_out_dev, n_out_cap, cin, cout, kvol, s);
  if (n_out_cap > 0 && cin % 16 == 0 && cout % 16 == 0 && cin <= 64 && cout <= 64 && (cin < 64 || cout < 64)) {
#define IG_SMALL(WNV, BKV)                                                                                                                          \
    return transpose_w ? launch_igemm_fwd<4, 1, IGEMM_SMALL_WM, WNV, false, BKV>(in, w, nbr, ld, out, n_out_dev, n_out_cap, cin, cout, kvol, s)   \
                       : launch_igemm_fwd<4, 1, IGEMM_SMALL_WM, WNV, true, BKV>(in, w, nbr, ld, out, n_out_dev, n_out_cap, cin, cout, kvol, s);
    if (cin == 16 || cin == 32) {
      if (cout == 16) { IG_SMALL(1, 32) }
      if (cout == 32) { IG_SMALL(2, 32) }
      if (cout == 64) { IG_SMALL(4, 32) }
    }
#undef IG_SMALL
  }
  if (cin % 64 != 0 || cout % 64 != 0 || cout < 64) return U3D_ERR_UNSUPPORTED;
  if (n_out_cap <= 0) return U3D_OK;
  if (transpose_w) return U3D_ERR_UNSUPPORTED;
#define IG_CASE(A, B, C, D) return launch_igemm_fwd<A, B, C, D, true>(in, w, nbr, ld, out, n_out_dev, n_out_cap, cin, cout, kvol, s);
  const long long wg256 = (long long)u3d_cdiv(n_out_cap, 256) * (cout / 256 > 0 ? cout / 256 : 1);
  if (cout % 256 == 0 && wg256 < 128) { IG_CASE(4, 2, 4, 4) }
  if (cout >= 256 && cout % 256 == 0) { IG_CASE(2, 4, 8, 4) }
  if (cout >= 128 && cout % 128 == 0) { IG_CASE(4, 2, 4, 4) }
  if (cout % 64 == 0) { IG_CASE(4, 1, 2, 4) }
#undef IG_CASE
  return U3D_ERR_UNSUPPORTED;
}
```

uni3detr_amd/native.py:

```python
import ctypes as C
import os

import numpy as np
import torch

from . import abi

_HERE = os.path.dirname(os.path.abspath(__file__))
LIB_PATH = os.environ.get("U3D_LIB_PATH") or os.path.join(_HERE, "libu3d_hip.so")

_ABI = abi.load()
_K = _ABI.constants


def _struct(c_name, py_name):
    return abi.structure(_ABI.structs[c_name], py_name)


def _slot_names(prefix):
    names = sorted((v, n[len(prefix):]) for n, v in _K.items() if n.startswith(prefix))
    assert [v for v, _ in names] == list(range(len(names))) and names[-1][1] == "COUNT" and _K[prefix + "COUNT"] == len(names) - 1
    return [n for _, n in names[:-1]]


U3D_ERR_UNSUPPORTED = _K["U3D_ERR_UNSUPPORTED"]
F32, BF16 = _K["U3D_F32"], _K["U3D_BF16"]


class U3DError(RuntimeError):
    pass


BitGridStruct = _struct("u3d_bitgrid", "BitGridStruct")

for _n, _v in _K.items():
    if _n.startswith(("U3D_DL_", "U3D_DLN_")):
        globals()[_n[4:]] = _v
DS_NAMES = _slot_names("U3D_DS_")
DG_NAMES = _slot_names("U3D_DG_")
DecLayerParams = _struct("u3d_declayer_params", "DecLayerParams")
DecLayerDims = _struct("u3d_declayer_dims", "DecLayerDims")
WPackDesc = _struct("u3d_wpack_desc", "WPackDesc")

_lib = None
_I3 = C.c_int32 * 3
_F3 = C.c_float * 3
_F6 = C.c_float * 6


def exported_symbols():
    return sorted(_ABI.prototypes)


def lib():
    global _lib
    if _lib is None:
        if not os.path.exists(LIB_PATH):
            raise U3DError(f"{LIB_PATH} is missing: run `python -m uni3detr_amd.build` (hipcc, gfx950). "
                           "There is no CPU/PyTorch fallback for the HIP hot path.")
        l = C.CDLL(LIB_PATH)
        for name, (res, args) in _ABI.prototypes.items():
            fn = getattr(l, name)
            fn.restype = res
            fn.argtypes = args
        _lib = l
    return _lib


def _check(rc, what):
    if rc != 0:
        raise U3DError(f"{what} failed: {lib().u3d_strerror(rc).decode()} ({rc})")


def _stream():
    return C.c_void_p(torch.cuda.current_stream().cuda_stream)


def _ptr(t):
    if t is None:
        return None
    assert t.is_cuda and t.is_contiguous(), "device-contiguous tensor required"
    return C.c_void_p(t.data_ptr())


def dtype_code(t):
    if t.dtype == torch.float32:
        return F32
    if t.dtype == torch.bfloat16:
        return BF16
    raise U3DError(f"unsupported dtype {t.dtype}")


class BitGrid:

    def __init__(self, batch, dims, device, linear=False):
        self.batch, self.dims = int(batch), tuple(int(d) for d in dims)
        self.linear = bool(linear)
        self.nwords = int(lib().u3d_bitgrid_nwords_layout(self.batch, *self.dims, 1 if linear else 0))
        self.words = torch.zeros(self.nwords, dtype=torch.int64, device=device)
        self.prefix = torch.empty(self.nwords + 1, dtype=torch.int32, device=device)
        self._scratch = torch.empty(int(lib().u3d_bitgrid_scan_scratch(self.nwords)), dtype=torch.int32, device=device)
        self.c = BitGridStruct(self.words.data_ptr(), self.prefix.data_ptr(), self.batch, *self.dims, 1 if linear else 0, 0)

    def set_row_capacity(self, cap):
        self.c.row_capacity = int(cap)

    def mark(self, coors):
        _check(lib().u3d_bitgrid_mark(C.byref(self.c), _ptr(coors), coors.shape[0], _stream()), "bitgrid_mark")

    def mark_strided(self, in_coors, n_dev, ksize, stride, pad):
        _check(lib().u3d_bitgrid_mark_strided(C.byref(self.c), _ptr(in_coors), _ptr(n_dev), in_coors.shape[0],
                                              _I3(*ksize), _I3(*stride), _I3(*pad), _stream()), "bitgrid_mark_strided")

    def scan(self):
        _check(lib().u3d_bitgrid_scan(C.byref(self.c), _ptr(self._scratch), _stream()), "bitgrid_scan")

    @property
    def count_dev(self):
        return self.prefix[self.nwords:]

    def rank(self, coors):
        out = torch.empty(coors.shape[0], dtype=torch.int32, device=coors.device)
        _check(lib().u3d_bitgrid_rank(C.byref(self.c), _ptr(coors), coors.shape[0], _ptr(out), _stream()), "bitgrid_rank")
        return out

    def coords(self, n):
        out = torch.empty((n, 4), dtype=torch.int32, device=self.words.device)
        _check(lib().u3d_bitgrid_coords(C.byref(self.c), _ptr(out), n, _stream()), "bitgrid_coords")
        return out

    def nbr_table(self, q_coors, n_dev, ksize, stride, pad, mode):
        n = q_coors.shape[0]
        ld = (n + 127) // 128 * 128
        kvol = ksize[0] * ksize[1] * ksize[2]
        nbr = torch.empty((kvol, ld), dtype=torch.int32, device=q_coors.device)
        _check(lib().u3d_nbr_table(C.byref(self.c), _ptr(q_coors), _ptr(n_dev), n, _I3(*ksize), _I3(*stride), _I3(*pad),
                                   mode, _ptr(nbr), ld, _stream()), "nbr_table")
        return nbr


def dense_nbr_table(batch, q_dims, t_dims, ksize, stride, pad, mode, device):
    n = batch * q_dims[0] * q_dims[1] * q_dims[2]
    ld = (n + 127) // 128 * 128
    kvol = ksize[0] * ksize[1] * ksize[2]
    nbr = torch.empty((kvol, ld), dtype=torch.int32, device=device)
    with torch.cuda.device(device):
        _check(lib().u3d_dense_nbr_table(batch, _I3(*q_dims), _I3(*t_dims), _I3(*ksize), _I3(*stride), _I3(*pad), mode, _ptr(nbr), ld,
                                         _stream()), "dense_nbr_table")
    return nbr


def voxelize_hard(points, scene_off, batch, max_pts_per_scene, voxel_size, pc_range, max_points, max_voxels,
                  want_voxels=True, want_mean=True):
    n_total, nfeat = points.shape
    cap = batch * max_voxels
    dev = points.device
    voxels = torch.empty((cap, max_points, nfeat), dtype=torch.float32, device=dev) if want_voxels else None
    coors = torch.full((cap, 4), -1, dtype=torch.int32, device=dev)
    num = torch.zeros((cap,), dtype=torch.int32, device=dev)
    mean = torch.zeros((cap, nfeat), dtype=torch.float32, device=dev) if want_mean else None
    voxel_off = torch.empty((batch + 1,), dtype=torch.int32, device=dev)
    wsb = int(lib().u3d_voxelize_hard_workspace(n_total, batch, max_pts_per_scene))
    ws = torch.empty(wsb, dtype=torch.uint8, device=dev)
    _check(lib().u3d_voxelize_hard(_ptr(points), _ptr(scene_off), batch, n_total, max_pts_per_scene, nfeat,
                                   _F3(*voxel_size), _F6(*pc_range), max_points, max_voxels, _ptr(voxels), _ptr(coors),
                                   _ptr(num), _ptr(mean), _ptr(voxel_off), _ptr(ws), wsb, _stream()), "voxelize_hard")
    return voxels, coors, num, mean, voxel_off


def voxelize_dynamic(points, scene_off, batch, voxel_size, pc_range):
    n_total, nfeat = points.shape
    coors = torch.empty((n_total, 4), dtype=torch.int32, device=points.device)
    _check(lib().u3d_voxelize_dynamic(_ptr(points), _ptr(scene_off), batch, n_total, nfeat, _F3(*voxel_size), _F6(*pc_range),
                                      _ptr(coors), _stream()), "voxelize_dynamic")
    return coors


def scatter_mean(points, rank, n_voxels):
    n_total, nfeat = points.shape
    sums = torch.zeros((n_voxels, nfeat), dtype=torch.float32, device=points.device)
    counts = torch.zeros((n_voxels,), dtype=torch.int32, device=points.device)
    _check(lib().u3d_scatter_mean(_ptr(points), _ptr(rank), n_total, nfeat, _ptr(sums), _ptr(counts), n_voxels, _stream()), "scatter_mean")
    return sums, counts


class ExternalEvent:

    def __init__(self):
        h = C.c_void_p()
        _check(lib().u3d_event_create(C.byref(h)), "event_create")
        self.h = h

    def record(self):
        _check(lib().u3d_event_record(self.h, 1, _stream()), "event_record")

    def elapsed_time(self, other):
        ms = C.c_float()
        _check(lib().u3d_event_elapsed_ms(self.h, other.h, C.byref(ms)), "event_elapsed_ms")
        return float(ms.value)

    def __del__(self):
        try:
            lib().u3d_event_destroy(self.h)
        except Exception:
            pass


class KernelTimer:

    def __init__(self, mode="time", targets=(), per_step=0):
        self.mode, self.calls, self.census = mode, [], []
        self.targets, self.per_step, self.counter, self.marks = set(targets), per_step, 0, {}

    def begin(self):
        if self.mode == "off":
            return None
        if self.mode == "mark":
            i = self.counter % self.per_step if self.per_step else self.counter
            self.counter += 1
            if i not in self.targets:
                return None
            try:
                e = ExternalEvent()
                e.record()
            except U3DError:
                self.mode, self.marks = "off", {}
                return None
            return (i, e)
        e = torch.cuda.Event(enable_timing=True)
        e.record()
        return e

    def end(self, tag, e0, meta=None):
        if self.mode == "off":
            return
        if self.mode == "mark":
            if e0 is not None:
                try:
                    e1 = ExternalEvent()
                    e1.record()
                    self.marks[e0[0]] = (tag, e0[1], e1)
                except U3DError:
                    self.mode, self.marks = "off", {}
            return
        e1 = torch.cuda.Event(enable_timing=True)
        e1.record()
        self.calls.append((tag, e0, e1))
        if self.mode == "census":
            self.census.append((tag, meta))

    def mark_durations_ms(self):
        torch.cuda.synchronize()
        return {i: a.elapsed_time(b) for i, (t, a, b) in self.marks.items()}

    def durations_ms(self):
        torch.cuda.synchronize()
        return [(t, a.elapsed_time(b)) for t, a, b in self.calls]


TIMER = None
CALL_KIND = "sparse"
USE_IGEMM_V2 = True


def census_meta(n_in, n_out, cin, cout, kvol, nbr, act_bytes=2, w_bytes=None, v2=True, split=False):
    if split:
        act_bytes = w_bytes = 4
    elif w_bytes is None:
        w_bytes = act_bytes
    tab = nbr.t if isinstance(nbr, RevNbr) else nbr
    pairs = n_out if tab is None else int((tab[:kvol, :n_out] >= 0).sum().item())
    meta = dict(kind=CALL_KIND, v2=v2, split=True) if split else dict(kind=CALL_KIND, v2=v2)
    meta.update(n_in=n_in, n_out=n_out, cin=cin, cout=cout, kvol=kvol, pairs=pairs,
                bytes=n_in * cin * act_bytes + n_out * cout * act_bytes + 8 * pairs + kvol * cin * cout * w_bytes, flops=2 * pairs * cin * cout)
    return meta


def timed_begin():
    t = TIMER
    return None if t is None else (t, t.begin())


def timed_end(region, tag, *shape, **price):
    if region is not None:
        t, e0 = region
        t.end(tag, e0, census_meta(*shape, **price) if (shape and t.mode == "census") else None)


def fwd_stats_layout(n_out, cin, cout, kvol, has_nbr):
    p, r = C.c_int32(0), C.c_int32(0)
    if lib().u3d_igemm_fwd_stats_layout(n_out, cin, cout, kvol, int(has_nbr), C.byref(p), C.byref(r)) != 0:
        return None
    return p.value, r.value


def spconv_fwd_stats(inp, w_nmajor, nbr, n_out_dev, n_out, cout):
    cin, kvol = inp.shape[1], w_nmajor.shape[0]
    if inp.dtype != torch.bfloat16 or not USE_IGEMM_V2 or (nbr is None and kvol != 1):
        return None
    layout = fwd_stats_layout(n_out, cin, cout, kvol, nbr is not None)
    if layout is None or layout[0] == 0:
        return None
    nblocks, tr = layout
    out = torch.empty((n_out, cout), dtype=inp.dtype, device=inp.device)
    stats = torch.empty((nblocks, 2, cout), dtype=torch.float64, device=inp.device)
    ld = nbr.shape[1] if nbr is not None else 0
    region = timed_begin()
    _check(lib().u3d_igemm_fwd_stats_bf16(_ptr(inp), _ptr(w_nmajor), _ptr(nbr), ld, _ptr(out), _ptr(n_out_dev), n_out, cin, cout, kvol,
                                          _ptr(stats), _stream()), "igemm_fwd_stats_bf16")
    if region is not None:
        timed_end(region, "spconv_fwd", inp.shape[0], n_out, cin, cout, kvol, nbr)
    return out, stats, tr


class BnEpi(_struct("u3d_bn_epi", "_BnEpi")):

    @staticmethod
    def of(x, y, mean, invstd, gamma, beta, relu):
        p = lambda t: None if t is None else t.data_ptr()
        return BnEpi(p(x), p(y), p(mean), p(invstd), p(gamma), p(beta), int(relu), 0)


def spconv_dgrad_bnstats(dout, w_nmajor, nbr, n_dev, n, cout, addend, epi):
    kvol, cin = w_nmajor.shape[0], dout.shape[1]
    if dout.dtype != torch.bfloat16 or not USE_IGEMM_V2 or nbr is None:
        return None
    layout = fwd_stats_layout(n, cin, cout, kvol, True)
    if layout is None or layout[1] == 0:
        return None
    nblocks, tr = layout
    out = torch.empty((n, cout), dtype=dout.dtype, device=dout.device)
    stats = torch.empty((nblocks, 2, cout), dtype=torch.float64, device=dout.device)
    nbr_p, ld = _nbr_ptr_ld(nbr)
    region = timed_begin()
    rc = lib().u3d_igemm_dgrad_bnstats_bf16(_ptr(dout), _ptr(w_nmajor), nbr_p, ld, _ptr(addend), _ptr(out), _ptr(n_dev), n, cin, cout, kvol,
                                            C.byref(epi), _ptr(stats), _stream())
    if rc == U3D_ERR_UNSUPPORTED:
        return None
    _check(rc, "igemm_dgrad_bnstats_bf16")
    if region is not None:
        timed_end(region, "spconv_dgrad", dout.shape[0], n, cin, cout, kvol, nbr)
    return out, stats, tr


def bn_bwd_finalize_partials(partial, tile_rows, n_dev, n_cap):
    nb, _, c = partial.shape
    sums = torch.empty((2, c), dtype=torch.float64, device=partial.device)
    s32 = torch.empty((2, c), dtype=torch.float32, device=partial.device)
    _check(lib().u3d_bn_bwd_finalize_partials(_ptr(partial), nb, tile_rows, _ptr(n_dev), n_cap, c, _ptr(sums), _ptr(s32), _stream()),
           "bn_bwd_finalize_partials")
    return sums, s32


class SubmHalo:
    TILE = 128

    MAX_ROWS = 140 * 256 * 32

    def __init__(self, nbr_fwd, n_dev, n_cap):
        dev = nbr_fwd.device
        a, b, t = C.c_int64(0), C.c_int64(0), C.c_int32(0)
        _check(lib().u3d_subm_halo_sizes(n_cap, C.byref(a), C.byref(b), C.byref(t)), "subm_halo_sizes")
        self.tiles, self.n_dev, self.n_cap, self.nbr = t.value, n_dev, n_cap, nbr_fwd
        self.kvol = nbr_fwd.shape[0]
        self.tile_rows = torch.empty((a.value,), dtype=torch.int32, device=dev)
        self.loc = torch.empty((b.value,), dtype=torch.int16, device=dev)
        self.tile_cnt = torch.empty((t.value,), dtype=torch.int32, device=dev)
        rc = lib().u3d_subm_halo_build(_ptr(nbr_fwd), nbr_fwd.shape[1], _ptr(n_dev), n_cap, _ptr(self.tile_rows), _ptr(self.loc),
                                       _ptr(self.tile_cnt), self.kvol, _stream())
        self.ok = rc != U3D_ERR_UNSUPPORTED
        if self.ok:
            _check(rc, "subm_halo_build")


def subm_halo_wgrad(x, dy, halo, out=None, max_slots=0):
    assert x.dtype == torch.bfloat16 and dy.dtype == torch.bfloat16 and x.shape == dy.shape == (halo.n_cap, 64)
    dw = out.view(27, 64, 64) if (out is not None and out.is_contiguous() and out.dtype == torch.float32 and out.numel() == 27 * 4096) \
        else torch.empty((27, 64, 64), dtype=torch.float32, device=x.device)
    wsb = int(lib().u3d_subm_halo_wgrad64_workspace())
    ws = torch.empty(wsb, dtype=torch.uint8, device=x.device)
    region = timed_begin()
    _check(lib().u3d_subm_halo_wgrad64_bf16(_ptr(x), _ptr(dy), _ptr(halo.tile_rows), _ptr(halo.loc), _ptr(halo.tile_cnt), _ptr(halo.n_dev),
                                            halo.n_cap, _ptr(dw), _ptr(ws), wsb, int(max_slots), _stream()), "subm_halo_wgrad64_bf16")
    if region is not None:
        timed_end(region, "spconv_wgrad", halo.n_cap, halo.n_cap, 64, 64, 27, halo.nbr, w_bytes=4)
    return dw


def subm_halo_wpack(w_nmajor, out=None):
    k, c = w_nmajor.shape[0], w_nmajor.shape[1]
    assert w_nmajor.dtype == torch.bfloat16 and w_nmajor.is_contiguous() and w_nmajor.shape[2] == c
    assert (k == 27 and c == 64) or (1 <= k <= 27 and c == 128)
    out = torch.empty_like(w_nmajor) if out is None else out
    if c == 64:
        _check(lib().u3d_subm_halo_wpack(_ptr(w_nmajor), _ptr(out), _stream()), "subm_halo_wpack")
    else:
        _check(lib().u3d_subm_halo_wpack128(_ptr(w_nmajor), _ptr(out), k, _stream()), "subm_halo_wpack128")
    return out


def subm_halo_wpack_plan(pairs, device):
    k, c = pairs[0][0].shape[0], pairs[0][0].shape[1]
    assert all(tuple(a.shape) == (k, c, c) for a, _ in pairs) and ((k == 27 and c == 64) or c == 128)
    src = torch.tensor([a.data_ptr() for a, _ in pairs], dtype=torch.int64, device=device)
    dst = torch.tensor([b.data_ptr() for _, b in pairs], dtype=torch.int64, device=device)
    return src, dst, len(pairs), pairs, c, k


def subm_halo_wpack_batched(plan):
    if plan[4] == 64:
        _check(lib().u3d_subm_halo_wpack_batched(_ptr(plan[0]), _ptr(plan[1]), plan[2], _stream()), "subm_halo_wpack_batched")
    else:
        _check(lib().u3d_subm_halo_wpack128_batched(_ptr(plan[0]), _ptr(plan[1]), plan[2], plan[5], _stream()), "subm_halo_wpack128_batched")


def subm_halo_conv(inp, w_packed, halo, krev=False, addend=None, want_stats=False, tag="spconv_fwd", bn_epi=None, max_slots=0):
    c = inp.shape[1]
    assert inp.dtype == torch.bfloat16 and c in (64, 128) and tuple(w_packed.shape) == (halo.kvol, c, c) and inp.shape[0] == halo.n_cap
    assert c == 128 or halo.kvol == 27
    assert c == 64 or bn_epi is None, "the BatchNorm-backward epilogue exists on the 64-channel kernel only"
    out = torch.empty_like(inp)
    stats = torch.empty((halo.tiles, 2, c), dtype=torch.float64, device=inp.device) if want_stats else None
    region = timed_begin()
    if c == 64:
        _check(lib().u3d_subm_halo_conv64_bf16(_ptr(inp), _ptr(w_packed), _ptr(halo.tile_rows), _ptr(halo.loc), _ptr(halo.tile_cnt),
                                               _ptr(halo.n_dev), halo.n_cap, int(krev), _ptr(addend), _ptr(out), _ptr(stats),
                                               None if bn_epi is None else C.byref(bn_epi), int(max_slots), _stream()),
               "subm_halo_conv64_bf16")
    else:
        _check(lib().u3d_subm_halo_conv128_bf16(_ptr(inp), _ptr(w_packed), _ptr(halo.tile_rows), _ptr(halo.loc), _ptr(halo.tile_cnt),
                                                _ptr(halo.n_dev), halo.n_cap, int(krev), _ptr(addend), _ptr(out), _ptr(stats),
                                                int(max_slots), halo.kvol, _stream()), "subm_halo_conv128_bf16")
    if region is not None:
        timed_end(region, tag, halo.n_cap, halo.n_cap, c, c, halo.kvol, halo.nbr)
    return (out, stats, SubmHalo.TILE) if want_stats else out


def subm_halo_conv_affine(inp, w_packed, halo, shift, relu, addend=None, max_slots=0, out=None, tag="spconv_fwd"):
    c = inp.shape[1]
    assert inp.dtype == torch.bfloat16 and c in (64, 128) and tuple(w_packed.shape) == (halo.kvol, c, c) and inp.shape[0] == halo.n_cap
    assert w_packed.dtype == torch.bfloat16 and (c == 128 or halo.kvol == 27)
    assert shift.dtype == torch.float32 and tuple(shift.shape) == (c,) and shift.data_ptr() % 16 == 0
    assert addend is None or (addend.dtype == torch.bfloat16 and addend.shape == inp.shape)
    if out is None:
        out = torch.empty_like(inp)
    assert out.shape == inp.shape and out.dtype == torch.bfloat16
    region = timed_begin()
    if c == 64:
        _check(lib().u3d_subm_halo_conv64_affine_bf16(_ptr(inp), _ptr(w_packed), _ptr(halo.tile_rows), _ptr(halo.loc), _ptr(halo.tile_cnt),
                                                      _ptr(halo.n_dev), halo.n_cap, _ptr(addend), _ptr(out), _ptr(shift), int(bool(relu)),
                                                      int(max_slots), _stream()), "subm_halo_conv64_affine_bf16")
    else:
        _check(lib().u3d_subm_halo_conv128_affine_bf16(_ptr(inp), _ptr(w_packed), _ptr(halo.tile_rows), _ptr(halo.loc), _ptr(halo.tile_cnt),
                                                       _ptr(halo.n_dev), halo.n_cap, _ptr(addend), _ptr(out), _ptr(shift), int(bool(relu)),
                                                       int(max_slots), halo.kvol, _stream()), "subm_halo_conv128_affine_bf16")
    if region is not None:
        timed_end(region, tag, halo.n_cap, halo.n_cap, c, c, halo.kvol, halo.nbr)
    return out


def bn_finalize_partials(stats, tile_rows, n_dev, n_cap, eps, momentum, running_mean=None, running_var=None, num_batches=None):
    nblocks, _, c = stats.shape
    mean = torch.empty((c,), dtype=torch.float32, device=stats.device)
    invstd = torch.empty((c,), dtype=torch.float32, device=stats.device)
    _check(lib().u3d_bn_finalize_partials(_ptr(stats), nblocks, tile_rows, _ptr(n_dev), n_cap, c, eps, momentum, _ptr(running_mean),
                                          _ptr(running_var), _ptr(num_batches), _ptr(mean), _ptr(invstd), _stream()), "bn_finalize_partials")
    return mean, invstd


class RevNbr:

    def __init__(self, table):
        self.t = table
        self.shape = table.shape

    def ptr_ld(self):
        k, ld = self.t.shape
        return C.c_void_p(self.t.data_ptr() + (k - 1) * ld * 4), -ld


def _nbr_ptr_ld(nbr):
    if nbr is None:
        return _ptr(None), 0
    if isinstance(nbr, RevNbr):
        return nbr.ptr_ld()
    return _ptr(nbr), nbr.shape[1]


def spconv_fwd(inp, w, nbr, n_out_dev, n_out, cout, transpose_w=False, tag=None, addend=None):
    kvol = w.shape[0]
    cin = inp.shape[1]
    out = torch.empty((n_out, cout), dtype=inp.dtype, device=inp.device)
    nbr_p, ld = _nbr_ptr_ld(nbr)
    region = timed_begin()
    rc = U3D_ERR_UNSUPPORTED
    if addend is not None and inp.dtype == torch.bfloat16 and USE_IGEMM_V2 and ld != 0 and addend.dtype == torch.bfloat16 \
            and addend.shape == out.shape and addend.is_contiguous():
        rc = lib().u3d_igemm_fwd_add_bf16(_ptr(inp), _ptr(w), nbr_p, ld, _ptr(addend), _ptr(out), _ptr(n_out_dev), n_out, cin, cout, kvol,
                                          1 if transpose_w else 0, _stream())
        if rc not in (0, U3D_ERR_UNSUPPORTED):
            _check(rc, "igemm_fwd_add_bf16")
        if rc == 0:
            addend = None
    if rc == U3D_ERR_UNSUPPORTED and inp.dtype == torch.bfloat16 and USE_IGEMM_V2:
        rc = lib().u3d_igemm_fwd_bf16(_ptr(inp), _ptr(w), nbr_p, ld, _ptr(out), _ptr(n_out_dev), n_out, cin, cout, kvol,
                                      1 if transpose_w else 0, _stream())
        if rc not in (0, U3D_ERR_UNSUPPORTED):
            _check(rc, "igemm_fwd_bf16")
    if rc == U3D_ERR_UNSUPPORTED:
        _check(lib().u3d_spconv_fwd(_ptr(inp), _ptr(w), nbr_p, ld, _ptr(out), _ptr(n_out_dev), n_out, cin, cout, kvol,
                                    1 if transpose_w else 0, dtype_code(inp), _stream()), "spconv_fwd")
    if region is not None:
        timed_end(region, tag or ("spconv_dgrad" if transpose_w else "spconv_fwd"), inp.shape[0], n_out, cin, cout, kvol, nbr,
                  act_bytes=inp.element_size(), v2=bool(rc == 0))
    if addend is not None:
        out += addend
    return out


def split_rows(x, n_dev, n_cap=None):
    n_cap = x.shape[0] if n_cap is None else n_cap
    assert x.dtype == torch.float32 and x.is_contiguous()
    out = torch.empty((2 * n_cap, x.shape[1]), dtype=torch.bfloat16, device=x.device)
    _check(lib().u3d_split_rows_f32(_ptr(x), _ptr(n_dev), n_cap, x.shape[1], _ptr(out), _stream()), "split_rows_f32")
    return out


def direct_serves(cin, cout, kvol):
    return kvol == 27 and cin in (16, 32, 64) and cout in (16, 32, 64) and not (cin == 64 and cout == 64)


def spconv_fwd_split_direct(xs, w3, nbr, n_out_dev, n_out, cout, tag="spconv_fwd"):
    cin, n_in = xs.shape[1], xs.shape[0] // 2
    out = torch.empty((n_out, cout), dtype=torch.float32, device=xs.device)
    nbr_p, ld = _nbr_ptr_ld(nbr)
    region = timed_begin()
    _check(lib().u3d_igemm_direct_split_bf16(_ptr(xs), _ptr(w3), nbr_p, ld, _ptr(out), _ptr(n_out_dev), n_out, n_in, cin, cout, _stream()),
           "igemm_direct_split_bf16")
    if region is not None:
        timed_end(region, tag, n_in, n_out, cin, cout, 27, nbr, split=True)
    return out


_SplitRowsJobs = _struct("U3dSplitRowsJobs", "_SplitRowsJobs")


def split_rows_batch_into(tensors, outs):
    for i in range(0, len(tensors), 32):
        jobs = _SplitRowsJobs()
        chunk = list(zip(tensors[i:i + 32], outs[i:i + 32]))
        jobs.njobs = len(chunk)
        for j, (t, o) in enumerate(chunk):
            assert t.dtype == torch.float32 and t.dim() == 2 and t.stride(1) == 1 and t.shape[1] % 4 == 0 and t.stride(0) % 4 == 0
            assert o.dtype == torch.bfloat16 and o.is_contiguous() and tuple(o.shape) == (2 * t.shape[0], t.shape[1])
            jobs.src[j], jobs.dst[j] = t.data_ptr(), o.data_ptr()
            jobs.ld[j], jobs.rows[j], jobs.cols[j] = t.stride(0), t.shape[0], t.shape[1]
        _check(lib().u3d_split_rows_batch(C.byref(jobs), _stream()), "split_rows_batch")


def split_rows_batch(tensors):
    outs = [torch.empty((2 * t.shape[0], t.shape[1]), dtype=torch.bfloat16, device=t.device) for t in tensors]
    split_rows_batch_into(tensors, outs)
    return outs


def sum3(a, b, c):
    assert a.shape == b.shape == c.shape and a.dtype == b.dtype == c.dtype == torch.float32
    a, b, c = a.contiguous(), b.contiguous(), c.contiguous()
    if a.numel() % 4 != 0 or not a.is_cuda:
        return a + b + c
    out = torch.empty_like(a)
    _check(lib().u3d_sum3_f32(_ptr(a), _ptr(b), _ptr(c), _ptr(out), a.numel(), _stream()), "sum3_f32")
    return out


def _split3_geometry(w, layout, nmajor):
    if layout == "dhwio":
        kd, kh, kw, cin, cout = w.shape
        k = kd * kh * kw
        sk, s_ci, s_co = cin * cout, cout, 1
    else:
        cout, cin, kd, kh, kw = w.shape
        k = kd * kh * kw
        sk, s_ci, s_co = 1, k, cin * k
    a, b, sa, sb = (cout, cin, s_co, s_ci) if nmajor else (cin, cout, s_ci, s_co)
    return k, a, b, sk, sa, sb


class Split3Set:

    class _Job(C.Structure):
        _fields_ = [("src", C.c_void_p), ("dst", C.c_void_p), ("sk", C.c_int64), ("sa", C.c_int64), ("sb", C.c_int64),
                    ("K", C.c_int32), ("A", C.c_int32), ("B", C.c_int32), ("first_block", C.c_int32)]

    def __init__(self):
        self.entries = {}
        self.jobs_dev = None
        self._keep = []
        self.total_blocks = 0
        self.dirty = True
        self.fresh = False

    def get(self, weight, layout, nmajor):
        e = self.entries.get((weight.data_ptr(), bool(nmajor)))
        if e is not None and e[0]() is not None and e[1] == layout and e[7] == tuple(weight.shape):
            if self.fresh and e[5] and e[6] == weight._version:
                return e[3]
        return None

    def add(self, weight, layout, nmajor, dst):
        import weakref
        key = (weight.data_ptr(), bool(nmajor))
        old = self.entries.get(key)
        if old is not None and old[0]() is not None and old[1] == layout and old[7] == tuple(weight.shape) and old[5]:
            return
        self.entries[key] = [weakref.ref(weight), layout, bool(nmajor), dst, weight.data_ptr(), False, -1, tuple(weight.shape)]
        self.dirty = True

    def refresh(self):
        dead = [k for k, e in self.entries.items() if e[0]() is None]
        for k in dead:
            del self.entries[k]
            self.dirty = True
        moved = [k for k, e in self.entries.items() if e[0]().data_ptr() != e[4]]
        for k in moved:
            del self.entries[k]
            self.dirty = True
        if not self.entries:
            self.fresh = False
            return
        if self.dirty:
            if torch.cuda.is_current_stream_capturing():
                self.fresh = False
                return
            assert int(lib().u3d_split3_job_bytes()) == C.sizeof(Split3Set._Job)
            jobs = (Split3Set._Job * len(self.entries))()
            fb = 0
            for j, e in enumerate(self.entries.values()):
                w = e[0]().detach()
                k, a, b, sk, sa, sb = _split3_geometry(w, e[1], e[2])
                jobs[j].src, jobs[j].dst = w.data_ptr(), e[3].data_ptr()
                jobs[j].sk, jobs[j].sa, jobs[j].sb = sk, sa, sb
                jobs[j].K, jobs[j].A, jobs[j].B, jobs[j].first_block = k, a, b, fb
                fb += int(lib().u3d_split3_job_blocks(k, a, b))
                e[5] = True
            raw = torch.frombuffer(bytearray(bytes(jobs)), dtype=torch.uint8)
            dev = next(iter(self.entries.values()))[3].device
            self.jobs_dev = raw.to(dev)
            self._keep.append(self.jobs_dev)
# ... 1395 lines not shown
```

uni3detr_amd/plugin/dense.py:

```python

import numpy as np
import torch
from torch import nn

from .. import native as nv
from .. import sparse as sp
from ..registry import BACKBONES, NECKS


def _conv(cfg, cin, cout, kernel, stride=1, padding=0):
    cfg = dict(cfg)
    t = cfg.pop("type")
    if t != "Conv3d":
        raise NotImplementedError("the HIP dense path implements the Conv3d variant used by every shipped config")
    if cfg.get("bias", True):
        raise NotImplementedError("shipped configs build these convolutions with bias=False")
    return nn.Conv3d(cin, cout, kernel, stride=stride, padding=padding, **cfg)


def _norm(cfg, c):
    cfg = dict(cfg)
    t = cfg.pop("type")
    assert t == "BN3d", "shipped configs use BN3d"
    cfg.pop("requires_grad", None)
    return nn.BatchNorm3d(c, **cfg)


_BRANCH_STREAMS = []
PARALLEL_BRANCHES = True


class Lattice:

    _cache = {}

    @classmethod
    def conv(cls, device, batch, dims_in, ksize, stride, pad):
        key = ("c", str(device), batch, tuple(dims_in), tuple(ksize), tuple(stride), tuple(pad))
        g = cls._cache.get(key)
        if g is None:
            dims_out = tuple((d + 2 * p - k) // s + 1 for d, k, s, p in zip(dims_in, ksize, stride, pad))
            n_in = batch * dims_in[0] * dims_in[1] * dims_in[2]
            n_out = batch * dims_out[0] * dims_out[1] * dims_out[2]
            one = all(k == 1 for k in ksize) and all(s == 1 for s in stride)
            fwd = None if one else nv.dense_nbr_table(batch, dims_out, dims_in, ksize, stride, pad, 0, device)
            bwd = None if one else nv.dense_nbr_table(batch, dims_in, dims_out, ksize, stride, pad, 1, device)
            n_in_dev = torch.tensor([n_in], dtype=torch.int32, device=device)
            n_out_dev = torch.tensor([n_out], dtype=torch.int32, device=device)
            g = (sp.ConvGeom(fwd, bwd, n_in, n_in_dev, n_out, n_out_dev, kind="dense", strided=any(s > 1 for s in stride)), dims_out)
            cls._cache[key] = g
        return g

    @classmethod
    def upsample_index(cls, device, batch, dims_in, s):
        key = ("u", str(device), batch, tuple(dims_in), s)
        v = cls._cache.get(key)
        if v is None:
            D, H, W = dims_in
            b = torch.arange(batch, device=device).view(-1, 1, 1, 1)
            z = torch.arange(D, device=device).view(1, -1, 1, 1)
            y = torch.arange(H * s, device=device).view(1, 1, -1, 1)
            x = torch.arange(W * s, device=device).view(1, 1, 1, -1)
            in_row = ((b * D + z) * H + y // s) * W + x // s
            tap = (y % s) * s + (x % s)
            idx = (in_row * (s * s) + tap).reshape(-1).int().contiguous()
            inv = torch.empty_like(idx)
            inv[idx.long()] = torch.arange(idx.numel(), device=device, dtype=torch.int32)
            v = (idx, inv, (D, H * s, W * s))
            cls._cache[key] = v
        return v


FUSED_LEVEL_SUM = True
FUSED_UPSAMPLE_ORDER = True


class _GatherBijection(torch.autograd.Function):
    @staticmethod
    def forward(ctx, rows, idx, inv):
        ctx.save_for_backward(inv)
        return nv.gather_rows(rows.contiguous(), idx)

    @staticmethod
    def backward(ctx, dout):
        (inv,) = ctx.saved_tensors
        return nv.gather_rows(dout.contiguous(), inv), None, None


def to_rows(x):
    B, C, D, H, W = x.shape
    return x.permute(0, 2, 3, 4, 1).reshape(-1, C), B, (D, H, W)


def to_volume(rows, B, dims):
    return rows.view(B, *dims, rows.shape[1]).permute(0, 4, 1, 2, 3)


def conv_bn_relu(rows, B, dims, conv, bn, post_add=None, fan_token=None, bn_in=None, bn_out=None):
    ks, st, pd = tuple(conv.kernel_size), tuple(conv.stride), tuple(conv.padding)
    geom, dims_out = Lattice.conv(rows.device, B, dims, ks, st, pd)
    return sp.conv_bn(rows, conv.weight, geom, bn, geom.n_out_dev, None, True, "oidhw", post_add, fan_token=fan_token, bn_in=bn_in,
                      bn_out=bn_out), dims_out


def deconv_bn_relu(rows, B, dims, deconv, bn, post_add=None):
    s = deconv.stride[1]
    assert tuple(deconv.kernel_size) == (1, s, s) and tuple(deconv.stride) == (1, s, s), "non-overlapping (1,s,s) upsampling only"
    cin, cout = deconv.weight.shape[0], deconv.weight.shape[1]
    n_in = rows.shape[0]
    geom, _ = Lattice.conv(rows.device, B, dims, (1, 1, 1), (1, 1, 1), (0, 0, 0))
    w = deconv.weight.permute(0, 2, 3, 4, 1).reshape(1, 1, 1, cin, s * s * cout)
    y = sp.sparse_conv(rows, w, geom).view(n_in * s * s, cout)
    idx, inv, dims_out = Lattice.upsample_index(rows.device, B, dims, s)
    n_dev = Lattice.conv(rows.device, B, dims_out, (1, 1, 1), (1, 1, 1), (0, 0, 0))[0].n_out_dev
    if FUSED_UPSAMPLE_ORDER:
        return sp.bn_rows(y, bn, n_dev, None, True, row_map=inv, post_add=post_add), dims_out
    y = _GatherBijection.apply(y, idx, inv)
    return sp.bn_rows(y, bn, n_dev, None, True, post_add=post_add), dims_out


FANOUT_FUSION = True


@BACKBONES.register_module()
class SECOND3D(nn.Module):
    def __init__(self, in_channels=128, out_channels=[128, 128, 256], layer_nums=[3, 5, 5], layer_strides=[2, 2, 2],
                 is_cascade=True, norm_cfg=dict(type="BN3d", eps=1e-3, momentum=0.01), conv_cfg=dict(type="Conv3d", bias=False),
                 init_cfg=None, pretrained=None):
        super().__init__()
        assert len(layer_strides) == len(layer_nums) == len(out_channels)
        in_filters = list(in_channels) if isinstance(in_channels, (list, tuple)) else [in_channels, *out_channels[:-1]]
        self.is_cascade = is_cascade
        self.kernel_type = conv_cfg.type if hasattr(conv_cfg, "type") else conv_cfg["type"]
        kernel = tuple(conv_cfg.pop("kernel")) if "kernel" in conv_cfg else (1, 3, 3)
        padding = tuple((k - 1) // 2 for k in kernel)
        blocks = []
        for i, n in enumerate(layer_nums):
            s = layer_strides[i]
            layers = [_conv(conv_cfg, in_filters[i], out_channels[i], kernel, (1, s, s), padding), _norm(norm_cfg, out_channels[i]),
                      nn.ReLU(inplace=True)]
            for _ in range(n):
                layers += [_conv(conv_cfg, out_channels[i], out_channels[i], kernel, 1, padding), _norm(norm_cfg, out_channels[i]),
                           nn.ReLU(inplace=True)]
            blocks.append(nn.Sequential(*layers))
        self.blocks = nn.ModuleList(blocks)

    @staticmethod
    def _run_block(blk, rows, B, dims, fan=None):
        mods = list(blk)
        prev = None
        for j in range(0, len(mods), 3):
            cur = sp.BnGradToken() if j + 3 < len(mods) else None
            rows, dims = conv_bn_relu(rows, B, dims, mods[j], mods[j + 1], fan_token=fan if j == 0 else None, bn_in=prev, bn_out=cur)
            prev = cur
        return rows, dims

    def forward(self, x):
        rows, B, dims = to_rows(x)
        outs = []
        if self.is_cascade:
            for blk in self.blocks:
                rows, dims = self._run_block(blk, rows, B, dims)
                outs.append(to_volume(rows, B, dims))
            return tuple(outs)
        if not PARALLEL_BRANCHES or torch.cuda.is_current_stream_capturing():
            fan = sp.FanoutToken(len(self.blocks)) if (FANOUT_FUSION and rows.requires_grad and len(self.blocks) > 1) else None
            seq = [self._run_block(blk, rows, B, dims, fan) for blk in self.blocks]
            return tuple(to_volume(r, B, d) for r, d in seq)
        cur = torch.cuda.current_stream()
        while len(_BRANCH_STREAMS) < len(self.blocks) - 1:
            _BRANCH_STREAMS.append(torch.cuda.Stream())
        results = [None] * len(self.blocks)
        for i in range(len(self.blocks) - 1, 0, -1):
            st = _BRANCH_STREAMS[i - 1]
            st.wait_stream(cur)
            with torch.cuda.stream(st):
                results[i] = self._run_block(self.blocks[i], rows, B, dims)
        results[0] = self._run_block(self.blocks[0], rows, B, dims)
        for i in range(1, len(self.blocks)):
            rows.record_stream(_BRANCH_STREAMS[i - 1])
            cur.wait_stream(_BRANCH_STREAMS[i - 1])
        return tuple(to_volume(r, B, d) for r, d in results)


@NECKS.register_module()
class SECOND3DFPN(nn.Module):
    def __init__(self, in_channels=[128, 128, 256], out_channels=[256, 256, 256], upsample_strides=[1, 2, 4],
                 norm_cfg=dict(type="BN3d", eps=1e-3, momentum=0.01), upsample_cfg=dict(type="deconv3d", bias=False),
                 conv_cfg=dict(type="Conv3d", bias=False), extra_conv=None, use_conv_for_no_stride=False, use_for_distill=False,
                 init_cfg=None):
        super().__init__()
        assert len(out_channels) == len(upsample_strides) == len(in_channels)
        self.in_channels, self.out_channels = in_channels, out_channels
        self.fp16_enabled = False
        if use_for_distill:
            raise NotImplementedError("use_for_distill is not used by any shipped Uni3DETR config")
        assert upsample_cfg["type"] == "deconv3d" and not upsample_cfg.get("bias", True)
        deblocks = []
        for i, oc in enumerate(out_channels):
            s = upsample_strides[i]
            if s > 1 or (s == 1 and not use_conv_for_no_stride):
                up = nn.ConvTranspose3d(in_channels[i], oc, (1, s, s), stride=(1, s, s), bias=False)
# ... 37 lines not shown
```

uni3detr_amd/sparse.py:

```python
import collections
import contextlib
import os

import torch

from . import native as nv
from .shadow import conv_weights, halo_packs

K3, S1, P1 = (3, 3, 3), (1, 1, 1), (1, 1, 1)


class Level:

    def __init__(self, grid, coords, n, n_dev):
        self.grid, self.coords, self.n, self.n_dev = grid, coords, n, n_dev
        self.dims, self.batch = grid.dims, grid.batch
        self._subm = None
        self._halo = None

    def halo(self):
        if self._halo is None:
            h = nv.SubmHalo(self.subm_tables()[0], self.n_dev, self.n) if self.n <= nv.SubmHalo.MAX_ROWS else None
            self._halo = h if (h is not None and h.ok) else False
        return self._halo or None

    def subm_tables(self):
        if self._subm is None:
            fwd = self.grid.nbr_table(self.coords, self.n_dev, K3, S1, P1, 0)
            bwd = nv.RevNbr(fwd) if REV_SUBM_TABLE else self.grid.nbr_table(self.coords, self.n_dev, K3, S1, P1, 1)
            self._subm = (fwd, bwd)
        return self._subm


class ResidualToken:

    def __init__(self):
        self.dres = None


class BnGradToken:

    def __init__(self):
        self.epi = None
        self.keep = None
        self.partial = None
        self.c = 0

    def fill(self, x, y, mean, invstd, gamma, beta, relu):
        self.keep = (x, y, mean, invstd, gamma, beta)
        self.epi = nv.BnEpi.of(x, y, mean, invstd, gamma, beta, relu)
        self.c = x.shape[1]


class FanoutToken:

    def __init__(self, n):
        self.n = self.remaining = n
        self.acc = None

    def step(self, din):
        self.remaining -= 1
        if self.remaining > 0:
            self.acc = din
            return None
        self.acc, self.remaining = None, self.n
        return din


class ConvGeom:

    def __init__(self, nbr_fwd, nbr_bwd, n_in, n_in_dev, n_out, n_out_dev, kind="sparse", strided=False):
        self.strided = strided
        self.nbr_fwd, self.nbr_bwd = nbr_fwd, nbr_bwd
        self.n_in, self.n_in_dev, self.n_out, self.n_out_dev = n_in, n_in_dev, n_out, n_out_dev
        self.kind = kind
        self.level = None


def level_from_coors(coors, batch, dims):
    dev = coors.device
    g = nv.BitGrid(batch, dims, dev)
    g.mark(coors)
    g.scan()
    n = coors.shape[0]
    g.set_row_capacity(n)
    rank = g.rank(coors)
    lvl = Level(g, g.coords(n), n, g.count_dev)
    return lvl, rank


def subm_geom(lvl):
    fwd, bwd = lvl.subm_tables()
    g = ConvGeom(fwd, bwd, lvl.n, lvl.n_dev, lvl.n, lvl.n_dev)
    g.level = lvl
    return g


def strided_level(lvl, ksize, stride, pad, capacity=None):
    dims_out = tuple((d + 2 * p - k) // s + 1 for d, k, s, p in zip(lvl.dims, ksize, stride, pad))
    g = nv.BitGrid(lvl.batch, dims_out, lvl.coords.device)
    g.mark_strided(lvl.coords, lvl.n_dev, ksize, stride, pad)
    g.scan()
    n_out = int(g.count_dev.item()) if capacity is None else int(capacity)
    if capacity is not None:
        g.set_row_capacity(n_out)
    out = Level(g, g.coords(n_out), n_out, g.count_dev)
    fwd = lvl.grid.nbr_table(out.coords, out.n_dev, ksize, stride, pad, 0)
    bwd = g.nbr_table(lvl.coords, lvl.n_dev, ksize, stride, pad, 1)
    return out, ConvGeom(fwd, bwd, lvl.n, lvl.n_dev, n_out, out.n_dev, strided=True)


REV_SUBM_TABLE = True
SUBM_HALO = os.environ.get("U3D_SUBM_HALO", "1") == "1"
HALO_WGRAD = True
HALO_128 = True
STRIDED_DGRAD_SPLIT = True
NMAJOR_FWD = True
STRIDED_SPLIT_MIN_RATIO = 16
STRIDED_SPLIT_SPARSE_RATIO = 16


_CONV_USES = {}


def reset_conv_uses():
    _CONV_USES.clear()
    _PLANES_BWD.clear()


SPLIT_BF16 = os.environ.get("U3D_SPLIT_BF16", "1") == "1"
SPLIT_FUSED_ADD = True
_SPLIT = [False]


_PLANES = {}
_PLANES_BWD = {}
BN_PLANES = True


def _planes_of(feats, n_dev):
    ent = _PLANES.get(id(feats))
    if ent is not None and ent[0] is feats and ent[2] == feats._version:
        return ent[1]
    xs = nv.split_rows(feats.contiguous(), n_dev)
    if _SPLIT[0]:
        _PLANES[id(feats)] = (feats, xs, feats._version)
    return xs


def _give_planes(t, planes):
    if planes is not None and _SPLIT[0]:
        _PLANES[id(t)] = (t, planes, t._version)


def _give_bwd_planes(t, planes):
    if planes is not None:
        _PLANES_BWD[t.data_ptr()] = (t, planes, t._version)


def _bwd_planes_of(dout, n_dev):
    ent = _PLANES_BWD.pop(dout.data_ptr(), None)
    if (ent is not None and ent[0].numel() == dout.numel() and ent[0].dtype == dout.dtype and ent[2] == ent[0]._version
            and dout.dim() == 2 and dout.is_contiguous() and ent[0].is_contiguous()):
        return ent[1].view(2 * dout.shape[0], dout.shape[1])
    return nv.split_rows(dout.float() if dout.dtype != torch.float32 else dout, n_dev)


@contextlib.contextmanager
def split_scope(on=True, split3=None):
    prev, prev3 = _SPLIT[0], nv.SPLIT3_ACTIVE
    _SPLIT[0] = bool(on) and SPLIT_BF16
    _PLANES.clear()
    _PLANES_BWD.clear()
    if _SPLIT[0]:
        nv.SPLIT3_ACTIVE = split3 if split3 is not None else nv.SPLIT3_DEFAULT
        if nv.SPLIT3_BATCH:
            nv.SPLIT3_ACTIVE.refresh()
    try:
        yield
    finally:
        _SPLIT[0] = prev
        nv.SPLIT3_ACTIVE = prev3
        _PLANES.clear()


def _split_serves(feats, cin, cout, kvol=None):
    if not (_SPLIT[0] and feats.is_cuda and feats.dtype == torch.float32):
        return None
    if cin % 64 == 0 and cout % 64 == 0:
        return "wide"
    if nv.direct_serves(cin, cout, kvol):
        return "narrow"
    return None


def _split_table(geom, which, n_rows, plane):
    owner = geom.level if (geom.level is not None and which != "id") else geom
    cache = owner.__dict__.setdefault("_split_tables", {})
    key = (which, plane)
    if key not in cache:
        t = geom.nbr_bwd if which == "bwd" else (None if which == "id" else geom.nbr_fwd)
        if t is None:
            t = torch.arange(n_rows, dtype=torch.int32, device=geom.n_out_dev.device).view(1, -1)
        elif isinstance(t, nv.RevNbr):
            t = t.t.flip(0)
        lo = torch.where(t >= 0, t + plane, t)
        cache[key] = torch.cat([t, lo] if which == "wgrad" else [t, t, lo], 0).contiguous()
    return cache[key]


def _halo_of(geom, kvol, cin, cout):
    if not (SUBM_HALO and REV_SUBM_TABLE and geom.level is not None and kvol == 27 and cin == cout
            and (cin == 64 or (cin == 128 and HALO_128)) and geom.n_out >= 4096):
        return None
    return geom.level.halo()


_ConvRoute = collections.namedtuple("_ConvRoute", "split nmajor halo kvol cin cout strided_split")


def _conv_route(feats, kio_shape, geom):
    kvol, cin, cout = kio_shape[0] * kio_shape[1] * kio_shape[2], kio_shape[3], kio_shape[4]
    bf16 = feats.dtype == torch.bfloat16
    nmajor = NMAJOR_FWD and bf16 and ((cin % 64 == 0 and cout % 64 == 0) or nv.direct_serves(cin, cout, kvol))
    split = _split_serves(feats, cin, cout, kvol)
    if split == "narrow" and geom.nbr_fwd is None:
        split = None
    halo = _halo_of(geom, kvol, cin, cout) if (nmajor and not split) else None
    strided_split = bool(STRIDED_DGRAD_SPLIT and geom.strided and kvol > 1 and (bf16 or split == "wide") and cout % 64 == 0
                         and (kvol * cin) % 64 == 0
                         and geom.n_out * (STRIDED_SPLIT_SPARSE_RATIO if geom.kind == "sparse" else STRIDED_SPLIT_MIN_RATIO) <= geom.n_in)
    return _ConvRoute(split, nmajor, halo, kvol, cin, cout, strided_split)


def _pending_addend(ctx):
    tok, fan = ctx.res_token, ctx.fan_token
    dres = tok.dres if tok is not None else None
    facc = fan.acc if fan is not None else None
    if dres is not None and facc is not None:
        return dres + facc
    return facc if dres is None else dres


def _finish_din(ctx, din, taken):
    tok, fan = ctx.res_token, ctx.fan_token
    if din is not None and not taken:
        if fan is not None and fan.acc is not None:
            din += fan.acc
        if tok is not None and tok.dres is not None:
            din = din + tok.dres
    if tok is not None:
        tok.dres = None
    return fan.step(din) if (fan is not None and din is not None) else din


class _SparseConv(torch.autograd.Function):
    @staticmethod
    def forward(ctx, feats, weight, geom, layout, want_stats=False, res_token=None, fan_token=None, bn_in=None):
        ctx.set_materialize_grads(False)
        kio_shape = weight.shape if layout == "dhwio" else tuple(weight.shape[i] for i in (2, 3, 4, 1, 0))
        if feats.shape[1] != kio_shape[3]:
            raise ValueError(f"sparse conv: input has {feats.shape[1]} channels, weight expects {kio_shape[3]}")
        r = ctx.route = _conv_route(feats, kio_shape, geom)
        ctx.geom, ctx.layout = geom, layout
        ctx.res_token = res_token
        ctx.fan_token = fan_token if (fan_token is not None and feats.requires_grad) else None
        ctx.bn_in = bn_in if (BN_GRAD_FUSION and bn_in is not None and bn_in.epi is not None and feats.dtype == torch.bfloat16
                              and fan_token is None) else None
        _CONV_USES[id(weight)] = _CONV_USES.get(id(weight), 0) + 1
        ctx.weight_id = id(weight)
        ctx.grad_view = getattr(weight, "_u3d_grad_view", None)
        ctx.kio_shape, ctx.wdtype = kio_shape, weight.dtype
        nv.CALL_KIND = geom.kind
        out_args = (geom.n_out_dev, geom.n_out, r.cout)
        if r.split:
            xs = _planes_of(feats, geom.n_in_dev)
            saved = (xs, weight)
            ctx.split3 = nv.SPLIT3_ACTIVE
            w3 = nv.split3_weights(weight, layout, nmajor=True)
            if r.split == "narrow":
                res = nv.spconv_fwd_split_direct(xs, w3, geom.nbr_fwd, *out_args)
            else:
                res = nv.spconv_fwd_split(xs, w3, _split_table(geom, "fwd", geom.n_out, feats.shape[0]), *out_args, want_stats=want_stats)
        else:
            kio, koi = conv_weights(weight, layout, feats.dtype, want_koi=r.nmajor)
            saved = (feats, kio)
            nbr = geom.nbr_fwd if r.kvol > 1 else None
            if r.halo is not None:
                pk_fwd, ctx.pk_bwd = halo_packs(weight, kio, koi)
                res = nv.subm_halo_conv(feats, pk_fwd, r.halo, want_stats=want_stats)
            else:
                res = nv.spconv_fwd_stats(feats, koi, nbr, *out_args) if (want_stats and r.nmajor) else None
                if res is None and r.nmajor:
                    res = nv.spconv_fwd(feats, koi, nbr, *out_args, transpose_w=True, tag="spconv_fwd")
                elif res is None:
                    res = nv.spconv_fwd(feats, kio, nbr, *out_args)
        y, stats, tr = res if isinstance(res, tuple) else (res, None, 0)
        ctx.save_for_backward(*saved)
        if not want_stats:
            return y
        if stats is None:
            stats = torch.empty(0, dtype=torch.float64, device=feats.device)
        else:
            stats._u3d_tile_rows = tr
        ctx.mark_non_differentiable(stats)
        return y, stats

    @staticmethod
    def backward(ctx, dout, _dstats=None):
        feats, wc = ctx.saved_tensors
        if dout is None:
            return None, None, None, None, None, None, None, None
        r, g = ctx.route, ctx.geom
        dout = dout.contiguous()
        nv.CALL_KIND = g.kind
        want_din, want_dw = ctx.needs_input_grad[:2]
        din, dw, taken = None, None, False
        if r.split:
            dys = _bwd_planes_of(dout, g.n_out_dev)
            if want_dw:
                dw = _split_weight_grad(ctx, r, feats, dys)
            if want_din:
                din, taken = _split_input_grad(ctx, r, wc, dys)
        else:
            if want_dw:
                dw = _weight_grad(ctx, r, feats, dout)
            if want_din:
                din, taken = _input_grad(ctx, r, wc, dout)
        return _finish_din(ctx, din, taken), dw, None, None, None, None, None, None


def _weight_grad(ctx, r, feats, dout):
    g, kvol = ctx.geom, r.kvol
    nbr = g.nbr_fwd if kvol > 1 else None
    v2 = feats.dtype == torch.bfloat16 and nv.USE_IGEMM_V2 and r.cin % 16 == 0 and r.cout % 16 == 0 and ctx.wdtype == torch.float32
    gv = ctx.grad_view if (v2 and ctx.grad_view is not None and ctx.grad_view.is_contiguous()
                           and ctx.grad_view.dtype == torch.float32 and _CONV_USES.get(ctx.weight_id, 0) == 1) else None
    if ctx.layout == "oidhw" and v2:
        ks = ctx.kio_shape
        return nv.spconv_wgrad(feats, dout, nbr, g.n_out_dev, kvol, out_oik=True, out=gv).view(ks[4], ks[3], ks[0], ks[1], ks[2])
    if ctx.layout == "dhwio" and v2 and r.halo is not None and HALO_WGRAD and r.cin == 64:
        return nv.subm_halo_wgrad(feats, dout, r.halo, out=gv).view(ctx.kio_shape)
    if ctx.layout == "dhwio" and v2:
        return nv.spconv_wgrad(feats, dout, nbr, g.n_out_dev, kvol, out=gv).view(ctx.kio_shape)
    dw = nv.spconv_wgrad(feats, dout, nbr, g.n_out_dev, kvol).reshape(ctx.kio_shape).to(ctx.wdtype)
    return dw.permute(4, 3, 0, 1, 2) if ctx.layout == "oidhw" else dw


def _input_grad(ctx, r, wc, dout):
    g, kvol, cin, cout = ctx.geom, r.kvol, r.cin, r.cout
    nbr = g.nbr_bwd if kvol > 1 else None
    add = _pending_addend(ctx)
    fits = add is not None and add.dtype == dout.dtype and add.is_contiguous() and tuple(add.shape) == (g.n_in, cin)
    if r.strided_split:
        prod = nv.linear_bf16(dout, wc.view(kvol * cin, cout), None, False)
        fan = ctx.fan_token
        if not (fits and fan is not None and add is fan.acc):
            add = None
        return nv.tap_gather_sum(prod, nbr, g.n_in_dev, g.n_in, cin, kvol, addend=add), add is not None
    bt = ctx.bn_in
    if bt is not None and (bt.c != cin or not (add is None or fits)):
        bt = None
    if r.halo is not None:
        if cin != 64:
            bt = None
        if not fits:
            add = None
        pk = ctx.pk_bwd if ctx.pk_bwd is not None else nv.subm_halo_wpack(wc)
        din = nv.subm_halo_conv(dout, pk, r.halo, krev=True, addend=add, want_stats=bt is not None, tag="spconv_dgrad",
                                bn_epi=None if bt is None else bt.epi)
        if bt is not None:
            din, st, tr = din
            bt.partial = (st, tr)
        return din, add is not None
    res = nv.spconv_dgrad_bnstats(dout, wc, nbr, g.n_in_dev, g.n_in, cin, add, bt.epi) if (bt is not None and kvol > 1) else None
    if res is not None:
        bt.partial = (res[1], res[2])
        return res[0], True
    return nv.spconv_fwd(dout, wc, nbr, g.n_in_dev, g.n_in, cin, transpose_w=True, addend=add), True


def _split_weight_grad(ctx, r, xs, dys):
    g, kvol = ctx.geom, r.kvol
    n_in, n_out = xs.shape[0] // 2, dys.shape[0] // 2
    if r.split == "narrow":
        xh, xl, dyh, dyl = xs[:n_in], xs[n_in:], dys[:n_out], dys[n_out:]
        parts = [nv.spconv_wgrad(x, dy, g.nbr_fwd, g.n_out_dev, kvol) for x, dy in ((xh, dyh), (xl, dyh), (xh, dyl))]
    else:
        ta = _split_table(g, "wgrad", n_out, n_in)
        a = nv.spconv_wgrad(xs, dys[:n_out], ta, g.n_out_dev, 2 * kvol)
        b = nv.spconv_wgrad(xs, dys[n_out:], ta[:kvol], g.n_out_dev, kvol)
        parts = [a[:kvol], a[kvol:], b]
    dwk = nv.sum3(*parts).reshape(ctx.kio_shape).to(ctx.wdtype)
    return dwk.permute(4, 3, 0, 1, 2) if ctx.layout == "oidhw" else dwk


def _split_input_grad(ctx, r, wc, dys):
    g, kvol, cin, cout = ctx.geom, r.kvol, r.cin, r.cout
    n_out = dys.shape[0] // 2
    w3 = nv.split3_weights(wc, ctx.layout, nmajor=False, cache=ctx.split3)
    if r.split == "narrow":
        return nv.spconv_fwd_split_direct(dys, w3, g.nbr_bwd, g.n_in_dev, g.n_in, cin, tag="spconv_dgrad"), False
    if r.strided_split:
        tid = _split_table(g, "id", n_out, n_out)
        wt3 = w3.view(3, kvol * cin, cout)
        prod = nv.spconv_fwd_split(dys, wt3, tid, g.n_out_dev, n_out, kvol * cin, tag="spconv_dgrad")
        return nv.tap_gather_sum(prod, g.nbr_bwd, g.n_in_dev, g.n_in, cin, kvol), False
    add = _pending_addend(ctx) if SPLIT_FUSED_ADD else None
    if add is not None and not (add.dtype == torch.float32 and add.is_contiguous() and tuple(add.shape) == (g.n_in, cin)):
        add = None
    t3 = _split_table(g, "bwd", g.n_in, n_out)
    return nv.spconv_fwd_split(dys, w3, t3, g.n_in_dev, g.n_in, cin, tag="spconv_dgrad", addend=add), add is not None


def sparse_conv(feats, weight, geom, layout="dhwio", fan_token=None):
    return _SparseConv.apply(feats, weight, geom, layout, False, None, fan_token)


BN_GRAD_FUSION = False
FUSED_CONV_STATS = True


_FOLD = [None]


@contextlib.contextmanager
def fold_scope(table):
    prev = _FOLD[0]
    _FOLD[0] = table
    try:
        yield
    finally:
        _FOLD[0] = prev


def conv_affine(feats, w_folded, shift, geom, relu=True):
    if torch.is_grad_enabled() and (feats.requires_grad or w_folded.requires_grad):
        raise RuntimeError("conv_affine is an inference path: it records no autograd node")
    if feats.dtype != torch.bfloat16 or not feats.is_cuda:
        raise RuntimeError(f"conv_affine needs bf16 device rows, got {feats.dtype} on {feats.device}")
    kvol, cin = w_folded.shape[0], w_folded.shape[2]
    if feats.shape[1] != cin:
        raise ValueError(f"conv_affine: input has {feats.shape[1]} channels, folded weight expects {cin}")
    nv.CALL_KIND = geom.kind
    nbr = geom.nbr_fwd if kvol > 1 else None
    return nv.igemm_fwd_affine(feats.contiguous(), w_folded, nbr, shift, relu, geom.n_out_dev, geom.n_out)


def conv_folded(feats, ent, geom, residual=None, relu=True):
    w_folded, shift, w_packed = ent
    kvol, cout, cin = w_folded.shape
    if torch.is_grad_enabled() and (feats.requires_grad or (residual is not None and residual.requires_grad)):
        raise RuntimeError("a folded conv + BatchNorm pair is an inference path: it records no autograd node")
    if feats.dtype != torch.bfloat16 or not feats.is_cuda:
        raise RuntimeError(f"a folded conv + BatchNorm pair needs bf16 device rows, got {feats.dtype} on {feats.device}")
    if feats.shape[1] != cin:
        raise ValueError(f"folded conv: input has {feats.shape[1]} channels, folded weight expects {cin}")
    if residual is not None and not (residual.dtype == torch.bfloat16 and tuple(residual.shape) == (geom.n_out, cout)):
        raise ValueError("folded conv: the residual must be bf16 rows of the output's shape")
    halo = _halo_of(geom, kvol, cin, cout) if w_packed is not None else None
    if halo is not None:
        nv.CALL_KIND = geom.kind
        return nv.subm_halo_conv_affine(feats.contiguous(), w_packed, halo, shift, relu, None if residual is None else residual.contiguous())
    if nv.direct_serves(cin, cout, kvol) and geom.nbr_fwd is not None:
        nv.CALL_KIND = geom.kind
        return nv.igemm_direct_affine(feats.contiguous(), w_folded, geom.nbr_fwd, shift, relu, geom.n_out_dev, geom.n_out,
                                      None if residual is None else residual.contiguous())
    if residual is None:
        return conv_affine(feats, w_folded, shift, geom, relu)
    return None


def conv_bn(feats, weight, geom, bn, n_dev, residual=None, relu=True, layout="dhwio", post_add=None, res_take=None, res_give=None,
            fan_token=None, bn_in=None, bn_out=None):
    if _FOLD[0] is not None:
        ent = _FOLD[0].get(id(bn))
        if ent is not None:
            if len(ent) == 2:
                if bn.training or residual is not None or post_add is not None:
                    raise RuntimeError("a folded conv + BatchNorm pair was called in training mode, or with a residual / level sum")
                return conv_affine(feats, ent[0], ent[1], geom, relu)
            if bn.training or post_add is not None:
                raise RuntimeError("a folded conv + BatchNorm pair of a sparse level was called in training mode, or with a level sum")
            y = conv_folded(feats, ent, geom, residual, relu)
            if y is not None:
                return y
    if FUSED_CONV_STATS and bn.training and feats.is_cuda and (feats.dtype == torch.bfloat16 or _split_serves(feats, feats.shape[1], bn.num_features) == "wide"):
        y, stats = _SparseConv.apply(feats, weight, geom, layout, True, res_take, fan_token, bn_in)
        if stats.numel():
            tr = getattr(stats, "_u3d_tile_rows", None)
            if tr is None:
                nb = stats.shape[0]
                tr = next((t for t in (128, 256, 192) if (y.shape[0] + t - 1) // t == nb), 0)
            return _BNRows.apply(y, bn.weight, bn.bias, residual, n_dev, bn, relu, True, stats, tr, None, post_add, res_give, bn_out)
        return _BNRows.apply(y, bn.weight, bn.bias, residual, n_dev, bn, relu, bn.training, None, 0, None, post_add, res_give, bn_out)
    return bn_rows(sparse_conv(feats, weight, geom, layout, fan_token), bn, n_dev, residual, relu, None, post_add)


class _BNRows(torch.autograd.Function):

    @staticmethod
    def forward(ctx, x, gamma, beta, residual, n_dev, bn, relu, training, stats=None, tile_rows=0, row_map=None, post_add=None, res_token=None,
                bn_tok=None):
        n = x.shape[0]
        if training and stats is not None:
            mean, invstd = nv.bn_finalize_partials(stats, tile_rows, n_dev, n, bn.eps, bn.momentum if bn.momentum is not None else 0.1,
                                                   bn.running_mean, bn.running_var, bn.num_batches_tracked)
        elif training:
            mean, invstd = nv.bn_forward_stats(x, n_dev, bn.eps, bn.momentum if bn.momentum is not None else 0.1,
                                               bn.running_mean, bn.running_var, bn.num_batches_tracked)
        else:
            mean = bn.running_mean
            invstd = torch.rsqrt(bn.running_var + bn.eps)
        g32, b32 = gamma.float(), beta.float()
        if post_add is not None:
            assert relu and residual is None and post_add.shape == x.shape and post_add.dtype == x.dtype
            post_add = post_add.contiguous()
        ctx.planes = bool(BN_PLANES and _SPLIT[0] and x.is_cuda and x.dtype == torch.float32 and x.shape[1] % 16 == 0)
        if ctx.planes:
            y, ypl = nv.bn_apply(x, mean, invstd, g32, b32, residual, relu, n_dev, row_map, post_add, want_planes=True)
            _give_planes(y, ypl)
        else:
            y = nv.bn_apply(x, mean, invstd, g32, b32, residual, relu, n_dev, row_map, post_add)
        ctx.remask = bool(relu and residual is None)
        ctx.save_for_backward(x, None if ctx.remask else y, mean, invstd, g32, b32)
        ctx.n_dev, ctx.relu, ctx.training, ctx.has_res = n_dev, relu, training, residual is not None
        ctx.pdtype = gamma.dtype
        ctx.row_map = row_map
        ctx.has_post = post_add is not None
        ctx.res_token = res_token if residual is not None else None
        ctx.bn_tok = None
        if bn_tok is not None and training and row_map is None and post_add is None and x.dtype == torch.bfloat16 and x.is_cuda:
# ... 65 lines not shown
```

Measured before the change: 436.5.

## Skip empty kernel taps per row tile in implicit-GEMM sparse conv

Adds a kernel that builds, for each 64-row block, a bitmask of the neighbor-table taps that have any valid entry. The glds8 256/192x256 implicit-GEMM body now iterates only over the live taps of its tile and advances through them with a ctz-based iterator instead of stage%kvol. The mask is computed once per cached dense geometry and used in the forward, forward-stats and dgrad paths. This is meant to remove MMA and load stages over taps that are all empty, such as boundary taps in dense strided layers, at the cost of an extra mask kernel and more index arithmetic inside the pipeline.

Result: no change. 436.2 (-0.1%).

```diff
diff --git a/include/u3d_hip.h b/include/u3d_hip.h
--- a/include/u3d_hip.h
+++ b/include/u3d_hip.h
@@ -59,6 +59,8 @@
 int32_t u3d_dense_nbr_table(int32_t batch, const int32_t q_dims[3], const int32_t t_dims[3], const int32_t ksize[3],
                             const int32_t stride[3], const int32_t pad[3], int32_t mode, int32_t* nbr, int32_t ld,
                             u3d_stream s);
+
+int32_t u3d_nbr_live_mask(const int32_t* nbr, int32_t ld, int32_t kvol, int32_t n_rows, uint32_t* live, u3d_stream s);
 
 int64_t u3d_voxelize_hard_workspace(int32_t n_total, int32_t batch, int32_t max_pts_per_scene);
 int32_t u3d_voxelize_hard(const float* points, const int32_t* scene_off, int32_t batch, int32_t n_total,
@@ -133,6 +135,10 @@
                                      const u3d_bn_epi* bn, double* stats, u3d_stream s);
 int32_t u3d_bn_bwd_finalize_partials(const double* partial, int32_t nblocks, int32_t rows_per_block, const int32_t* n_dev,
                                      int32_t n_cap, int32_t c, double* sums, float* sums_f32, u3d_stream s);
+int32_t u3d_igemm_fwd_live_plan(int32_t n_out_cap, int32_t cin, int32_t cout, int32_t kvol, int32_t* rows);
+int32_t u3d_igemm_fwd_live_bf16(const void* in, const void* w, const int32_t* nbr, int32_t ld, const uint32_t* live, const void* addend,
+                                void* out, const int32_t* n_out_dev, int32_t n_out_cap, int32_t cin, int32_t cout, int32_t kvol,
+                                const u3d_bn_epi* bn, double* stats, u3d_stream s);
 int32_t u3d_subm_halo_sizes(int32_t n_cap, int64_t* tile_rows_elems, int64_t* loc_elems, int32_t* tiles);
 int32_t u3d_subm_halo_build(const int32_t* nbr, int32_t ld, const int32_t* n_dev, int32_t n_cap, int32_t* tile_rows,
                             uint16_t* loc, int32_t* tile_cnt, int32_t kvol, u3d_stream s);
diff --git a/uni3detr_amd/csrc/geometry.hip b/uni3detr_amd/csrc/geometry.hip
--- a/uni3detr_amd/csrc/geometry.hip
+++ b/uni3detr_amd/csrc/geometry.hip
@@ -364,6 +364,27 @@
   return U3D_OK;
 }
 
+__global__ __launch_bounds__(256) void k_nbr_live_mask(const int* __restrict__ nbr, int ld, int kvol, int n_rows,
+                                                       unsigned* __restrict__ live) {
+  const int blk = blockIdx.x * 4 + (threadIdx.x >> 6), lane = threadIdx.x & 63;
+  if (blk * 64 >= n_rows) return;
+  const int row = blk * 64 + lane;
+  unsigned bits = 0;
+  for (int k = 0; k < kvol; ++k) {
+    const bool has = row < n_rows && nbr[(long long)k * ld + row] >= 0;
+    if (__ballot(has) != 0ull) bits |= 1u << k;
+  }
+  if (lane == 0) live[blk] = bits;
+}
+
+extern "C" int32_t u3d_nbr_live_mask(const int32_t* nbr, int32_t ld, int32_t kvol, int32_t n_rows, uint32_t* live, u3d_stream s) {
+  U3D_REQUIRE(nbr && live && kvol > 0 && kvol <= 27 && n_rows >= 0 && ld >= n_rows, U3D_ERR_ARG);
+  if (n_rows == 0) return U3D_OK;
+  hipLaunchKernelGGL(k_nbr_live_mask, dim3(u3d_cdiv(u3d_cdiv(n_rows, 64), 4)), dim3(256), 0, s, nbr, ld, kvol, n_rows, live);
+  U3D_CHECK_LAUNCH();
+  return U3D_OK;
+}
+
 __global__ void k_gather_rows(const uint32_t* __restrict__ in, const int* __restrict__ idx, int n, int row_words,
                               uint32_t* __restrict__ out) {
   long long t = (long long)blockIdx.x * blockDim.x + threadIdx.x;
diff --git a/uni3detr_amd/csrc/igemm_bf16.hip b/uni3detr_amd/csrc/igemm_bf16.hip
--- a/uni3detr_amd/csrc/igemm_bf16.hip
+++ b/uni3detr_amd/csrc/igemm_bf16.hip
@@ -452,7 +452,7 @@
 __device__ __forceinline__ void igemm_glds8_body(const u16* __restrict__ in, const u16* __restrict__ w, const int* __restrict__ nbr,
                                                  int ld, u16* __restrict__ out, const int* __restrict__ n_out_dev, int n_out_cap,
                                                  int cin, int cout, int kvol, const float* __restrict__ bias, int relu,
-                                                 double* __restrict__ stats, const BnEpi bn) {
+                                                 double* __restrict__ stats, const BnEpi bn, const unsigned* __restrict__ live) {
   constexpr int WAVES_M = 2, WAVES_N = 4, WM = 2 * RB, WN = 4, NW = 8;
   constexpr int BM = 64 * RB, BN = 256, BK = 64;
   constexpr int PIECE = 128 * BK;
@@ -467,7 +467,23 @@
   const int tid = threadIdx.x, lane = tid & 63;
   const int wv = __builtin_amdgcn_readfirstlane(tid >> 6);
   const int wm = wv / WAVES_N, wn = wv % WAVES_N;
-  const int nstage = kvol * (cin / BK);
+  const bool masked = live != nullptr;
+  unsigned lv = 0;
+  if (masked) {
+#pragma unroll
+    for (int j = 0; j < RB; ++j)
+      if (m0 + 64 * j < n_out_cap) lv |= live[tile * RB + j];
+    lv = __builtin_amdgcn_readfirstlane(lv & ((1u << kvol) - 1u));
+  }
+  const int kfirst = lv ? __builtin_ctz(lv) : 0;
+  const int nstage = (masked ? __builtin_popcount(lv) : kvol) * (cin / BK);
+  auto next_ktile = [&](int& kap, int& c0, bool go) {
+    const unsigned rest = masked ? (lv >> kap) >> 1 : 1u;
+    const int nk = kap + 1 + __builtin_ctz(rest | 0x80000000u);
+    const bool wrap = rest == 0 || nk >= kvol;
+    kap = go ? (wrap ? kfirst : nk) : kap;
+    c0 = go && wrap ? c0 + BK : c0;
+  };
 
   f32x4 acc[WM][WN];
 #pragma unroll
@@ -502,8 +518,8 @@
       mcl[sp][u] = m < n_out ? m : n_out - 1;
       idx_nxt[sp][u] = mcl[sp][u];
     }
-  auto load_idx_next = [&](int stage) {
-    const int* row = nbr + (long long)(stage % kvol) * ld;
+  auto load_idx_next = [&](int kap) {
+    const int* row = nbr + (long long)kap * ld;
 #pragma unroll
     for (int sp = 0; sp < 2; ++sp)
 #pragma unroll
@@ -515,8 +531,8 @@
 #pragma unroll
       for (int u = 0; u < 2; ++u) idx_cur[sp][u] = (arow[sp][u] >= 0 && m0 + arow[sp][u] < n_out) ? idx_nxt[sp][u] : -1;
   };
-  auto issue_a = [&](int st, int buf, int sp) {
-    const unsigned soff = (unsigned)((st / kvol) * BK) * 2u;
+  auto issue_a = [&](int c0, int buf, int sp) {
+    const unsigned soff = (unsigned)c0 * 2u;
     u16* dst = smem + buf * STAGE_ELEMS + sp * PIECE + wv * 1024;
 #pragma unroll
     for (int u = 0; u < 2; ++u) {
@@ -524,8 +540,8 @@
       __builtin_amdgcn_raw_ptr_buffer_load_lds(in_rs, (lds_void_ptr)(dst + u * 512), 16, voff, soff, 0, 0);
     }
   };
-  auto issue_b = [&](int st, int buf, int sp) {
-    const unsigned soff = (unsigned)((st % kvol) * cin * cout + (st / kvol) * BK) * 2u;
+  auto issue_b = [&](int kap, int c0, int buf, int sp) {
+    const unsigned soff = (unsigned)(kap * cin * cout + c0) * 2u;
     u16* dst = smem + buf * STAGE_ELEMS + (2 + sp) * PIECE + wv * 1024;
 #pragma unroll
     for (int u = 0; u < 2; ++u)
@@ -581,10 +597,14 @@
   }
 #define G8_VMCNT8() __builtin_amdgcn_s_waitcnt(0x0F78)
 
-  load_idx_next(0);
+  int k1 = kfirst, c1 = 0;
+  next_ktile(k1, c1, 1 < nstage);
+  int k2 = k1, c2 = c1;
+  next_ktile(k2, c2, 2 < nstage);
+  load_idx_next(kfirst);
   advance_idx();
-  issue_a(0, 0, 0); issue_b(0, 0, 0); issue_b(0, 0, 1); issue_a(0, 0, 1);
-  load_idx_next(1 < nstage ? 1 : 0);
+  issue_a(0, 0, 0); issue_b(kfirst, 0, 0, 0); issue_b(kfirst, 0, 0, 1); issue_a(0, 0, 1);
+  load_idx_next(k1);
   advance_idx();
   __builtin_amdgcn_s_waitcnt(0x0F70);
   G8_BAR();
@@ -594,27 +614,26 @@
   if (GLDS8_STAGGER && wm == 1) G8_BAR();
   for (int st = 0; st < nstage; ++st) {
     const int buf = st & 1;
-    const int nx = st + 1 < nstage ? st + 1 : st;
-    load_idx_next(st + 2 < nstage ? st + 2 : nstage - 1);
+    load_idx_next(k2);
     __builtin_amdgcn_sched_barrier(0);
     G8_READ_B(buf, 0)
 #if !GLDS8_BALANCE
     __builtin_amdgcn_sched_barrier(0);
     G8_READ_A(buf, 0)
 #endif
-    issue_a(nx, buf ^ 1, 0);
+    issue_a(c1, buf ^ 1, 0);
     G8_VMCNT8();
     G8_BAR();
     G8_MMA(0, 0)
     G8_BAR();
     G8_READ_B(buf, 1)
-    issue_b(nx, buf ^ 1, 0);
+    issue_b(k1, c1, buf ^ 1, 0);
     G8_VMCNT8();
     G8_BAR();
     G8_MMA(0, 1)
     G8_BAR();
     G8_READ_A(buf, 1)
-    issue_b(nx, buf ^ 1, 1);
+    issue_b(k1, c1, buf ^ 1, 1);
 #if GLDS8_BALANCE
     __builtin_amdgcn_s_waitcnt(0x0F74);
 #endif
@@ -624,7 +643,9 @@
 #if GLDS8_BALANCE
     G8_READ_A(buf ^ 1, 0)
 #endif
-    issue_a(nx, buf ^ 1, 1);
+    issue_a(c1, buf ^ 1, 1);
+    k1 = k2; c1 = c2;
+    next_ktile(k2, c2, st + 3 < nstage);
     __builtin_amdgcn_sched_barrier(0);
     advance_idx();
     __builtin_amdgcn_s_waitcnt(0x0F74);
@@ -647,23 +668,23 @@
 }
 __global__ __launch_bounds__(512) void k_igemm_glds8_256x256(const u16* in, const u16* w, const int* nbr, int ld, u16* out,
                                                              const int* n_out_dev, int n_out_cap, int cin, int cout, int kvol,
-                                                             const float* bias, int relu, double* stats, BnEpi bn) {
-  igemm_glds8_body(in, w, nbr, ld, out, n_out_dev, n_out_cap, cin, cout, kvol, bias, relu, stats, bn);
+                                                             const float* bias, int relu, double* stats, BnEpi bn, const unsigned* live) {
+  igemm_glds8_body(in, w, nbr, ld, out, n_out_dev, n_out_cap, cin, cout, kvol, bias, relu, stats, bn, live);
 }
 __global__ __launch_bounds__(512) void k_igemm_glds8_256x256_f32o(const u16* in, const u16* w, const int* nbr, int ld, u16* out,
                                                                   const int* n_out_dev, int n_out_cap, int cin, int cout, int kvol,
-                                                                  const float* bias, int relu, double* stats, BnEpi bn) {
-  igemm_glds8_body<true>(in, w, nbr, ld, out, n_out_dev, n_out_cap, cin, cout, kvol, bias, relu, stats, bn);
+                                                                  const float* bias, int relu, double* stats, BnEpi bn, const unsigned* live) {
+  igemm_glds8_body<true>(in, w, nbr, ld, out, n_out_dev, n_out_cap, cin, cout, kvol, bias, relu, stats, bn, live);
 }
 __global__ __launch_bounds__(512) void k_igemm_glds8_192x256(const u16* in, const u16* w, const int* nbr, int ld, u16* out,
                                                              const int* n_out_dev, int n_out_cap, int cin, int cout, int kvol,
-                                                             const float* bias, int relu, double* stats, BnEpi bn) {
-  igemm_glds8_body<false, 3>(in, w, nbr, ld, out, n_out_dev, n_out_cap, cin, cout, kvol, bias, relu, stats, bn);
+                                                             const float* bias, int relu, double* stats, BnEpi bn, const unsigned* live) {
+  igemm_glds8_body<false, 3>(in, w, nbr, ld, out, n_out_dev, n_out_cap, cin, cout, kvol, bias, relu, stats, bn, live);
 }
 __global__ __launch_bounds__(512) void k_igemm_glds8_192x256_f32o(const u16* in, const u16* w, const int* nbr, int ld, u16* out,
                                                                   const int* n_out_dev, int n_out_cap, int cin, int cout, int kvol,
-                                                                  const float* bias, int relu, double* stats, BnEpi bn) {
-  igemm_glds8_body<true, 3>(in, w, nbr, ld, out, n_out_dev, n_out_cap, cin, cout, kvol, bias, relu, stats, bn);
+                                                                  const float* bias, int relu, double* stats, BnEpi bn, const unsigned* live) {
+  igemm_glds8_body<true, 3>(in, w, nbr, ld, out, n_out_dev, n_out_cap, cin, cout, kvol, bias, relu, stats, bn, live);
 }
 static inline bool igemm_rows192(int n_out_cap, int col_blocks) {
   const long long w256 = (long long)u3d_cdiv(n_out_cap, 256) * col_blocks, w192 = (long long)u3d_cdiv(n_out_cap, 192) * col_blocks;
@@ -858,28 +879,28 @@
 }
 __global__ __launch_bounds__(512) void k_igemm_glds8_256x128(const u16* in, const u16* w, const int* nbr, int ld, u16* out,
                                                              const int* n_out_dev, int n_out_cap, int cin, int cout, int kvol,
-                                                             const float* bias, int relu, double* stats, BnEpi bn) {
+                                                             const float* bias, int relu, double* stats, BnEpi bn, const unsigned* live) {
   igemm_glds8n_body(in, w, nbr, ld, out, n_out_dev, n_out_cap, cin, cout, kvol, bias, relu, stats, bn);
 }
 __global__ __launch_bounds__(512) void k_igemm_glds8_256x128_f32o(const u16* in, const u16* w, const int* nbr, int ld, u16* out,
                                                                   const int* n_out_dev, int n_out_cap, int cin, int cout, int kvol,
-                                                                  const float* bias, int relu, double* stats, BnEpi bn) {
+                                                                  const float* bias, int relu, double* stats, BnEpi bn, const unsigned* live) {
   igemm_glds8n_body<true>(in, w, nbr, ld, out, n_out_dev, n_out_cap, cin, cout, kvol, bias, relu, stats, bn);
 }
 __global__ __launch_bounds__(512) void k_igemm_glds8_192x128(const u16* in, const u16* w, const int* nbr, int ld, u16* out,
                                                              const int* n_out_dev, int n_out_cap, int cin, int cout, int kvol,
-                                                             const float* bias, int relu, double* stats, BnEpi bn) {
+                                                             const float* bias, int relu, double* stats, BnEpi bn, const unsigned* live) {
   igemm_glds8n_body<false, 3>(in, w, nbr, ld, out, n_out_dev, n_out_cap, cin, cout, kvol, bias, relu, stats, bn);
 }
 __global__ __launch_bounds__(512) void k_igemm_glds8_192x128_f32o(const u16* in, const u16* w, const int* nbr, int ld, u16* out,
                                                                   const int* n_out_dev, int n_out_cap, int cin, int cout, int kvol,
-                                                                  const float* bias, int relu, double* stats, BnEpi bn) {
+                                                                  const float* bias, int relu, double* stats, BnEpi bn, const unsigned* live) {
   igemm_glds8n_body<true, 3>(in, w, nbr, ld, out, n_out_dev, n_out_cap, cin, cout, kvol, bias, relu, stats, bn);
 }
 #define U3D_GLDS_KERNEL(NAME, A, B, C, D)                                                                                        \
   __global__ __launch_bounds__(A* B * 64) void NAME(const u16* in, const u16* w, const int* nbr, int ld, u16* out,               \
                                                     const int* n_out_dev, int n_out_cap, int cin, int cout, int kvol,            \
-                                                    const float* bias, int relu, double* stats, BnEpi bn) {                      \
+                                                    const float* bias, int relu, double* stats, BnEpi bn, const unsigned* live) {                      \
     igemm_glds_body<A, B, C, D>(in, w, nbr, ld, out, n_out_dev, n_out_cap, cin, cout, kvol, bias, relu, stats, bn);               \
   }
 #define U3D_GLDS_KERNEL_X(NAME, ...) U3D_GLDS_KERNEL(NAME, __VA_ARGS__)
@@ -891,13 +912,14 @@
 #define U3D_GLDS_KERNEL_F32O(NAME, A, B, C, D)                                                                                   \
   __global__ __launch_bounds__(A* B * 64) void NAME(const u16* in, const u16* w, const int* nbr, int ld, u16* out,               \
                                                     const int* n_out_dev, int n_out_cap, int cin, int cout, int kvol,            \
-                                                    const float* bias, int relu, double* stats, BnEpi bn) {                      \
+                                                    const float* bias, int relu, double* stats, BnEpi bn, const unsigned* live) {                      \
     igemm_glds_body<A, B, C, D, true>(in, w, nbr, ld, out, n_out_dev, n_out_cap, cin, cout, kvol, bias, relu, stats, bn);         \
   }
 U3D_GLDS_KERNEL_F32O(k_igemm_glds_128x64_f32o, 4, 1, 2, 4)
 U3D_GLDS_KERNEL_F32O(k_igemm_glds_128x128_f32o, 2, 2, 4, 4)
 #undef U3D_GLDS_KERNEL_F32O
-typedef void (*glds_kernel_t)(const u16*, const u16*, const int*, int, u16*, const int*, int, int, int, int, const float*, int, double*, BnEpi);
+typedef void (*glds_kernel_t)(const u16*, const u16*, const int*, int, u16*, const int*, int, int, int, int, const float*, int, double*, BnEpi,
+                              const unsigned*);
 
 
 struct GldsKernel {
@@ -933,6 +955,7 @@
   size_t lds = 0;
   int partials = 0;
   bool served() const { return fn || direct.slot >= 0; }
+  bool takes_live() const { return glds == G8_256x256 || glds == G8_192x256; }
 };
 
 constexpr int GLDS8N_MIN_KTILES = 48;
@@ -976,12 +999,13 @@
 
 static int fwd_launch(const FwdPlan& p, const void* in, const void* w, const int32_t* nbr, int ld, void* out, const int32_t* n_out_dev,
                       int n_out_cap, int cin, int cout, int kvol, hipStream_t s, const void* bias = nullptr, int relu = 0,
-                      double* stats = nullptr, const BnEpi bn = BnEpi{}) {
+                      double* stats = nullptr, const BnEpi bn = BnEpi{}, const uint32_t* live = nullptr) {
+  if (live && !(p.takes_live() && kvol <= 27)) return U3D_ERR_UNSUPPORTED;
   if (p.direct.slot >= 0) return u3d_launch_igemm_direct(p.direct, in, w, nbr, ld, out, n_out_dev, n_out_cap, cin, cout, s, bias, stats);
   static unsigned long long lds_mask[G_COUNT][2] = {};
   if (p.lds > 64 * 1024) u3d_allow_lds_impl((const void*)p.fn, (int)p.lds, &lds_mask[p.glds][p.fn == GLDS_KERNELS[p.glds].f32]);
   hipLaunchKernelGGL(p.fn, p.grid, dim3(p.threads), p.lds, s, (const u16*)in, (const u16*)w, nbr, ld, (u16*)out, n_out_dev, n_out_cap, cin,
-                     cout, kvol, (const float*)bias, relu, stats, bn);
+                     cout, kvol, (const float*)bias, relu, stats, bn, (const unsigned*)live);
   return hipGetLastError() == hipSuccess ? U3D_OK : U3D_ERR_LAUNCH;
 }
 
@@ -1067,6 +1091,32 @@
   e.x = (const u16*)bn->x; e.y = (const u16*)bn->y; e.mean = bn->mean; e.invstd = bn->invstd; e.gamma = bn->gamma; e.beta = bn->beta;
   e.relu = bn->relu;
   return fwd_launch(p, in, w, nbr, ld, out, n_out_dev, n_out_cap, cin, cout, kvol, s, addend, addend ? 2 : 0, stats, e);
+}
+
+static FwdEpi live_epi(const void* addend, const u3d_bn_epi* bn, const double* stats) {
+  return bn ? EPI_BN_BWD : stats ? EPI_STATS : addend ? EPI_ADD : EPI_PLAIN;
+}
+extern "C" int32_t u3d_igemm_fwd_live_plan(int32_t n_out_cap, int32_t cin, int32_t cout, int32_t kvol, int32_t* rows) {
+  U3D_REQUIRE(rows, U3D_ERR_ARG);
+  const FwdPlan p = fwd_plan(n_out_cap, cin, cout, kvol, true, true, EPI_PLAIN);
+  if (!p.takes_live() || kvol > 27) return U3D_ERR_UNSUPPORTED;
+  *rows = p.rows;
+  return U3D_OK;
+}
+extern "C" int32_t u3d_igemm_fwd_live_bf16(const void* in, const void* w, const int32_t* nbr, int32_t ld, const uint32_t* live,
+                                           const void* addend, void* out, const int32_t* n_out_dev, int32_t n_out_cap, int32_t cin,
+                                           int32_t cout, int32_t kvol, const u3d_bn_epi* bn, double* stats, u3d_stream s) {
+  U3D_REQUIRE(in && w && nbr && live && out && n_out_dev && kvol > 0, U3D_ERR_ARG);
+  U3D_REQUIRE(!bn || (stats && bn->x && bn->mean && bn->invstd && (!bn->relu || bn->y || (bn->gamma && bn->beta))), U3D_ERR_ARG);
+  U3D_REQUIRE(bn || !(stats && addend), U3D_ERR_ARG);
+  const FwdPlan p = fwd_plan(n_out_cap, cin, cout, kvol, true, true, live_epi(addend, bn, stats));
+  if (!p.takes_live() || kvol > 27) return U3D_ERR_UNSUPPORTED;
+  BnEpi e;
+  if (bn) {
+    e.x = (const u16*)bn->x; e.y = (const u16*)bn->y; e.mean = bn->mean; e.invstd = bn->invstd; e.gamma = bn->gamma; e.beta = bn->beta;
+    e.relu = bn->relu;
+  }
+  return fwd_launch(p, in, w, nbr, ld, out, n_out_dev, n_out_cap, cin, cout, kvol, s, addend, addend ? 2 : 0, stats, e, live);
 }
 
 extern "C" int32_t u3d_igemm_fwd_bf16(const void* in, const void* w, const int32_t* nbr, int32_t ld, void* out,
diff --git a/uni3detr_amd/native.py b/uni3detr_amd/native.py
--- a/uni3detr_amd/native.py
+++ b/uni3detr_amd/native.py
@@ -148,6 +148,30 @@
         _check(lib().u3d_dense_nbr_table(batch, _I3(*q_dims), _I3(*t_dims), _I3(*ksize), _I3(*stride), _I3(*pad), mode, _ptr(nbr), ld,
                                          _stream()), "dense_nbr_table")
     return nbr
+
+
+def nbr_live_mask(nbr, n_rows):
+    kvol, ld = nbr.shape
+    live = torch.zeros(((n_rows + 63) // 64,), dtype=torch.int32, device=nbr.device)
+    with torch.cuda.device(nbr.device):
+        _check(lib().u3d_nbr_live_mask(_ptr(nbr), ld, kvol, n_rows, _ptr(live), _stream()), "nbr_live_mask")
+    return live
+
+
+class NbrLive:
+
+    def __init__(self, nbr, n_rows):
+        kvol = nbr.shape[0]
+        self.mask = nbr_live_mask(nbr, n_rows)
+        shifts = torch.arange(kvol, device=nbr.device, dtype=torch.int32).view(-1, 1)
+        self.counts = tuple(int(c) for c in ((self.mask.view(1, -1) >> shifts) & 1).sum(1).tolist())
+
+
+def fwd_live_rows(n_out, cin, cout, kvol):
+    rows = C.c_int32(0)
+    if not USE_IGEMM_V2 or lib().u3d_igemm_fwd_live_plan(n_out, cin, cout, kvol, C.byref(rows)) != 0:
+        return None
+    return rows.value
 
 
 def voxelize_hard(points, scene_off, batch, max_pts_per_scene, voxel_size, pc_range, max_points, max_voxels,
@@ -294,7 +318,12 @@
     return p.value, r.value
 
 
-def spconv_fwd_stats(inp, w_nmajor, nbr, n_out_dev, n_out, cout):
+def _fwd_live(what, inp, w, nbr, ld, live, addend, out, n_out_dev, n_out, cin, cout, kvol, epi, stats):
+    _check(lib().u3d_igemm_fwd_live_bf16(_ptr(inp), _ptr(w), _ptr(nbr), ld, _ptr(live), _ptr(addend), _ptr(out), _ptr(n_out_dev), n_out,
+                                         cin, cout, kvol, None if epi is None else C.byref(epi), _ptr(stats), _stream()), what + " (live)")
+
+
+def spconv_fwd_stats(inp, w_nmajor, nbr, n_out_dev, n_out, cout, live=None):
     cin, kvol = inp.shape[1], w_nmajor.shape[0]
     if inp.dtype != torch.bfloat16 or not USE_IGEMM_V2 or (nbr is None and kvol != 1):
         return None
@@ -306,8 +335,11 @@
     stats = torch.empty((nblocks, 2, cout), dtype=torch.float64, device=inp.device)
     ld = nbr.shape[1] if nbr is not None else 0
     region = timed_begin()
-    _check(lib().u3d_igemm_fwd_stats_bf16(_ptr(inp), _ptr(w_nmajor), _ptr(nbr), ld, _ptr(out), _ptr(n_out_dev), n_out, cin, cout, kvol,
-                                          _ptr(stats), _stream()), "igemm_fwd_stats_bf16")
+    if live is not None:
+        _fwd_live("igemm_fwd_stats_bf16", inp, w_nmajor, nbr, ld, live, None, out, n_out_dev, n_out, cin, cout, kvol, None, stats)
+    else:
+        _check(lib().u3d_igemm_fwd_stats_bf16(_ptr(inp), _ptr(w_nmajor), _ptr(nbr), ld, _ptr(out), _ptr(n_out_dev), n_out, cin, cout, kvol,
+                                              _ptr(stats), _stream()), "igemm_fwd_stats_bf16")
     if region is not None:
         timed_end(region, "spconv_fwd", inp.shape[0], n_out, cin, cout, kvol, nbr)
     return out, stats, tr
@@ -321,7 +353,7 @@
         return BnEpi(p(x), p(y), p(mean), p(invstd), p(gamma), p(beta), int(relu), 0)
 
 
-def spconv_dgrad_bnstats(dout, w_nmajor, nbr, n_dev, n, cout, addend, epi):
+def spconv_dgrad_bnstats(dout, w_nmajor, nbr, n_dev, n, cout, addend, epi, live=None):
     kvol, cin = w_nmajor.shape[0], dout.shape[1]
     if dout.dtype != torch.bfloat16 or not USE_IGEMM_V2 or nbr is None:
         return None
@@ -333,8 +365,12 @@
     stats = torch.empty((nblocks, 2, cout), dtype=torch.float64, device=dout.device)
     nbr_p, ld = _nbr_ptr_ld(nbr)
     region = timed_begin()
-    rc = lib().u3d_igemm_dgrad_bnstats_bf16(_ptr(dout), _ptr(w_nmajor), nbr_p, ld, _ptr(addend), _ptr(out), _ptr(n_dev), n, cin, cout, kvol,
-                                            C.byref(epi), _ptr(stats), _stream())
+    if live is not None:
+        _fwd_live("igemm_dgrad_bnstats_bf16", dout, w_nmajor, nbr, ld, live, addend, out, n_dev, n, cin, cout, kvol, epi, stats)
+        rc = 0
+    else:
+        rc = lib().u3d_igemm_dgrad_bnstats_bf16(_ptr(dout), _ptr(w_nmajor), nbr_p, ld, _ptr(addend), _ptr(out), _ptr(n_dev), n, cin, cout,
+                                                kvol, C.byref(epi), _ptr(stats), _stream())
     if rc == U3D_ERR_UNSUPPORTED:
         return None
     _check(rc, "igemm_dgrad_bnstats_bf16")
@@ -487,14 +523,21 @@
     return _ptr(nbr), nbr.shape[1]
 
 
-def spconv_fwd(inp, w, nbr, n_out_dev, n_out, cout, transpose_w=False, tag=None, addend=None):
+def spconv_fwd(inp, w, nbr, n_out_dev, n_out, cout, transpose_w=False, tag=None, addend=None, live=None):
     kvol = w.shape[0]
     cin = inp.shape[1]
     out = torch.empty((n_out, cout), dtype=inp.dtype, device=inp.device)
     nbr_p, ld = _nbr_ptr_ld(nbr)
     region = timed_begin()
     rc = U3D_ERR_UNSUPPORTED
-    if addend is not None and inp.dtype == torch.bfloat16 and USE_IGEMM_V2 and ld != 0 and addend.dtype == torch.bfloat16 \
+    fits = addend is not None and addend.dtype == torch.bfloat16 and addend.shape == out.shape and addend.is_contiguous()
+    if live is not None:
+        assert transpose_w and inp.dtype == torch.bfloat16 and USE_IGEMM_V2
+        _fwd_live("igemm_fwd_bf16", inp, w, nbr, ld, live, addend if fits else None, out, n_out_dev, n_out, cin, cout, kvol, None, None)
+        rc = 0
+        if fits:
+            addend = None
+    elif addend is not None and inp.dtype == torch.bfloat16 and USE_IGEMM_V2 and ld != 0 and addend.dtype == torch.bfloat16 \
             and addend.shape == out.shape and addend.is_contiguous():
         rc = lib().u3d_igemm_fwd_add_bf16(_ptr(inp), _ptr(w), nbr_p, ld, _ptr(addend), _ptr(out), _ptr(n_out_dev), n_out, cin, cout, kvol,
                                           1 if transpose_w else 0, _stream())
diff --git a/uni3detr_amd/plugin/dense.py b/uni3detr_amd/plugin/dense.py
--- a/uni3detr_amd/plugin/dense.py
+++ b/uni3detr_amd/plugin/dense.py
@@ -48,6 +48,10 @@
             n_in_dev = torch.tensor([n_in], dtype=torch.int32, device=device)
             n_out_dev = torch.tensor([n_out], dtype=torch.int32, device=device)
             g = (sp.ConvGeom(fwd, bwd, n_in, n_in_dev, n_out, n_out_dev, kind="dense", strided=any(s > 1 for s in stride)), dims_out)
+            if not one and len(fwd) <= 27:
+                lf, lb = nv.NbrLive(fwd, n_out), nv.NbrLive(bwd, n_in)
+                g[0].live_fwd = lf if min(lf.counts) < lf.mask.numel() else None
+                g[0].live_bwd = lb if min(lb.counts) < lb.mask.numel() else None
             cls._cache[key] = g
         return g
 
diff --git a/uni3detr_amd/sparse.py b/uni3detr_amd/sparse.py
--- a/uni3detr_amd/sparse.py
+++ b/uni3detr_amd/sparse.py
@@ -75,6 +75,7 @@
         self.n_in, self.n_in_dev, self.n_out, self.n_out_dev = n_in, n_in_dev, n_out, n_out_dev
         self.kind = kind
         self.level = None
+        self.live_fwd = self.live_bwd = None
 
 
 def level_from_coors(coors, batch, dims):
@@ -216,7 +217,16 @@
     return geom.level.halo()
 
 
-_ConvRoute = collections.namedtuple("_ConvRoute", "split nmajor halo kvol cin cout strided_split")
+_ConvRoute = collections.namedtuple("_ConvRoute", "split nmajor halo kvol cin cout strided_split live_fwd live_bwd", defaults=(False, False))
+
+
+def _live_of(geom, r):
+    lf, lb = getattr(geom, "live_fwd", None), getattr(geom, "live_bwd", None)
+    if not (r.nmajor and not r.split and r.halo is None and 1 < r.kvol <= 27):
+        return False, False
+    fwd = lf is not None and nv.fwd_live_rows(geom.n_out, r.cin, r.cout, r.kvol) is not None
+    bwd = lb is not None and not r.strided_split and nv.fwd_live_rows(geom.n_in, r.cout, r.cin, r.kvol) is not None
+    return fwd, bwd
 
 
 def _conv_route(feats, kio_shape, geom):
@@ -230,7 +240,9 @@
     strided_split = bool(STRIDED_DGRAD_SPLIT and geom.strided and kvol > 1 and (bf16 or split == "wide") and cout % 64 == 0
                          and (kvol * cin) % 64 == 0
                          and geom.n_out * (STRIDED_SPLIT_SPARSE_RATIO if geom.kind == "sparse" else STRIDED_SPLIT_MIN_RATIO) <= geom.n_in)
-    return _ConvRoute(split, nmajor, halo, kvol, cin, cout, strided_split)
+    r = _ConvRoute(split, nmajor, halo, kvol, cin, cout, strided_split)
+    live_fwd, live_bwd = _live_of(geom, r)
+    return r._replace(live_fwd=live_fwd, live_bwd=live_bwd)
 
 
 def _pending_addend(ctx):
@@ -290,9 +302,10 @@
                 pk_fwd, ctx.pk_bwd = halo_packs(weight, kio, koi)
                 res = nv.subm_halo_conv(feats, pk_fwd, r.halo, want_stats=want_stats)
             else:
-                res = nv.spconv_fwd_stats(feats, koi, nbr, *out_args) if (want_stats and r.nmajor) else None
+                live = geom.live_fwd.mask if r.live_fwd else None
+                res = nv.spconv_fwd_stats(feats, koi, nbr, *out_args, live=live) if (want_stats and r.nmajor) else None
                 if res is None and r.nmajor:
-                    res = nv.spconv_fwd(feats, koi, nbr, *out_args, transpose_w=True, tag="spconv_fwd")
+                    res = nv.spconv_fwd(feats, koi, nbr, *out_args, transpose_w=True, tag="spconv_fwd", live=live)
                 elif res is None:
                     res = nv.spconv_fwd(feats, kio, nbr, *out_args)
         y, stats, tr = res if isinstance(res, tuple) else (res, None, 0)
@@ -373,11 +386,12 @@
             din, st, tr = din
             bt.partial = (st, tr)
         return din, add is not None
-    res = nv.spconv_dgrad_bnstats(dout, wc, nbr, g.n_in_dev, g.n_in, cin, add, bt.epi) if (bt is not None and kvol > 1) else None
+    live = g.live_bwd.mask if r.live_bwd else None
+    res = nv.spconv_dgrad_bnstats(dout, wc, nbr, g.n_in_dev, g.n_in, cin, add, bt.epi, live=live) if (bt is not None and kvol > 1) else None
     if res is not None:
         bt.partial = (res[1], res[2])
         return res[0], True
-    return nv.spconv_fwd(dout, wc, nbr, g.n_in_dev, g.n_in, cin, transpose_w=True, addend=add), True
+    return nv.spconv_fwd(dout, wc, nbr, g.n_in_dev, g.n_in, cin, transpose_w=True, addend=add, live=live), True
 
 
 def _split_weight_grad(ctx, r, xs, dys):
```
